# xyang9527/dro-sfm

Measured on AMD Instinct MI355X. Metric: training images/sec (KITTI 192x640 mf self-sup), higher is better.
Workload: dtype f32; 1 GPU; KITTI 192x640 mf self-sup (configs[1]); model=DepthPoseNet it8-seq4-inter-out, global_batch=2, per_gpu_batch=2, ref_frames=2, parallelism=dp1, optimizer=Adam lr 2e-4, execution=hipgraph, update_blocks=depth block + pose block (side stream, with both context encoders), encoder_3x3_s1=hip, encoder_strided=hip, exchange=none (world 1)

## Files before the change

dro-sfm_amd/csrc/conv.hip:

```cpp
#include <hip/hip_runtime.h>

#include <algorithm>
#include <climits>
#include <cstddef>
#include <cstdio>
#include <cstdlib>
#include <cstring>
#include <map>
#include <mutex>
#include <string>
#include <type_traits>

#include "conv_common.hpp"
#include "dro_common.hpp"
#include "wgrad_group_plan.hpp"

namespace dro {


template <int BM, int MODE, int ACT, int EPI>
__global__ __launch_bounds__(256) void igemm_kernel(IgArgs a) {
  constexpr int WM = BM / 32;
  constexpr int KSTEPS = (WM == 2) ? 16 : 8;
  __shared__ float Ws[2][kBK][BM + 1];
// ... 179 lines not shown
    if (old == n - 1u) __hip_atomic_store(c, 0u, __ATOMIC_RELAXED, __HIP_MEMORY_SCOPE_AGENT);
  }
  __syncthreads();
  return *flag != 0u;
}

__device__ __forceinline__ void bn_put(double2* p, double a, double b) {
  double* q = reinterpret_cast<double*>(p);
  __hip_atomic_store(q, a, __ATOMIC_RELAXED, __HIP_MEMORY_SCOPE_AGENT);
  __hip_atomic_store(q + 1, b, __ATOMIC_RELAXED, __HIP_MEMORY_SCOPE_AGENT);
}

__device__ __forceinline__ double2 bn_get(const double2* p) {
  double* q = const_cast<double*>(reinterpret_cast<const double*>(p));
  return make_double2(__hip_atomic_load(q, __ATOMIC_RELAXED, __HIP_MEMORY_SCOPE_AGENT),
                      __hip_atomic_load(q + 1, __ATOMIC_RELAXED, __HIP_MEMORY_SCOPE_AGENT));
}

__device__ __forceinline__ double2 bn_fold(const double2* base, int n, int rows, int r, int j, int T) {
  double s1 = 0.0, s2 = 0.0;
  for (int p0 = j; p0 < n; p0 += 8 * T) {
    double2 v[8];
#pragma unroll
    for (int u = 0; u < 8; ++u) {
      const int p = p0 + u * T;
      v[u] = p < n ? bn_get(base + (size_t)p * rows + r) : make_double2(0.0, 0.0);
    }
#pragma unroll
    for (int u = 0; u < 8; ++u) {
      s1 += v[u].x;
      s2 += v[u].y;
    }
  }
  for (int o = 1; o < T; o <<= 1) {
    s1 += __shfl_xor(s1, o);
    s2 += __shfl_xor(s2, o);
  }
  return make_double2(s1, s2);
}

template <int EPI>
__device__ __forceinline__ void bn_finalize_row(const BnFuse& f, int r, int rows, long long L, double s1, double s2) {
  if (EPI == 5) {
    const double mean = s1 / (double)L;
    double var = s2 / (double)L - mean * mean;
    var = var > 0.0 ? var : 0.0;
    const float invstd = (float)(1.0 / sqrt(var + (double)f.eps));
    const float mu = (float)mean;
    f.coef[r] = (f.gamma ? f.gamma[r] : 1.f) * invstd;
    f.coef[rows + r] = mu;
    f.coef[2 * rows + r] = f.beta ? f.beta[r] : 0.f;
    f.save_mean[r] = mu;
    f.save_invstd[r] = invstd;
    if (f.rmean) {
      const double unb = L > 1 ? var * (double)L / (double)(L - 1) : var;
      f.rmean[r] = (1.f - f.momentum) * f.rmean[r] + f.momentum * mu;
      f.rvar[r] = (1.f - f.momentum) * f.rvar[r] + f.momentum * (float)unb;
    }
    if (r == 0 && f.nbt) *f.nbt += 1;
  } else {
    const float invstd = f.invstd[r];
    f.coef[r] = (f.gamma ? f.gamma[r] : 1.f) * invstd;
    f.coef[rows + r] = (float)(s1 / (double)L);
    f.coef[2 * rows + r] = (float)(s2 / (double)L);
    f.coef[3 * rows + r] = f.mean[r];
    f.coef[4 * rows + r] = invstd;
    if (f.dgamma) f.dgamma[r] = (float)s2;
    if (f.dbeta) f.dbeta[r] = (float)s1;
  }
}

template <int EPI>
__device__ void bn_finish(const IgArgs& a, int pt, int rt, int row0, int bm) {
  __shared__ unsigned flag;
  const BnFuse& f = a.bn;
  if (f.dbg & 1) return;
  const int rows = a.rows, ptiles = a.g.B * a.tiles_img;
  const int grp = pt / f.g1, lo = grp * f.g1, n1 = min(f.g1, ptiles - lo);
  if (!last_arrival(f.cnt + (size_t)rt * f.ngroups + grp, (unsigned)n1, &flag)) return;
  const int T = (int)blockDim.x / bm, rl = (int)threadIdx.x / T, j = (int)threadIdx.x - rl * T;
  const int r = row0 + rl;
  const bool live = r < rows;
  {
    const double2 v = bn_fold(f.part + (size_t)lo * rows, live ? n1 : 0, rows, live ? r : 0, j, T);
    if (live && j == 0) bn_put(f.part2 + (size_t)grp * rows + r, v.x, v.y);
  }
  if (!last_arrival(f.cnt + (size_t)a.row_tiles * f.ngroups + rt, (unsigned)f.ngroups, &flag)) return;
  const double2 v = bn_fold(f.part2, live ? f.ngroups : 0, rows, live ? r : 0, j, T);
  if (!live || j != 0) return;
  bn_finalize_row<EPI>(f, r, rows, (long long)a.g.B * a.g.H * a.g.W, v.x, v.y);
}

template <int EPI>
__global__ __launch_bounds__(256) void bn_finalize_kernel(BnFuse f, int rows, int ptiles, long long L) {
  __shared__ double red[2][4];
  const int r = blockIdx.x;
  double s1 = 0.0, s2 = 0.0;
  for (int p = threadIdx.x; p < ptiles; p += 256) {
    const double2 v = f.part[(size_t)p * rows + r];
    s1 += v.x;
    s2 += v.y;
  }
#pragma unroll
  for (int o = 32; o > 0; o >>= 1) {
    s1 += __shfl_xor(s1, o);
    s2 += __shfl_xor(s2, o);
  }
  const int w = threadIdx.x >> 6;
  if ((threadIdx.x & 63) == 0) {
    red[0][w] = s1;
    red[1][w] = s2;
  }
  __syncthreads();
  if (threadIdx.x == 0)
    bn_finalize_row<EPI>(f, r, rows, L, (red[0][0] + red[0][1]) + (red[0][2] + red[0][3]),
                         (red[1][0] + red[1][1]) + (red[1][2] + red[1][3]));
}

template <int BM, int KH, int KW, int MODE, int ACT, int EPI, int KS, int XF = 0>
__global__ __launch_bounds__(256 * KS) void dconv_kernel(IgArgs a) {
  using S = HaloShape<BM, KH, KW>;
  {
    const unsigned long long t0 = __builtin_amdgcn_s_memtime();
    if (a.stamps && (threadIdx.x == 0 || threadIdx.x == blockDim.x - 64))
      a.stamps[(size_t)blockIdx.x * 16 + (threadIdx.x == 0 ? 10 : 11)] = t0;
  }
  constexpr int PF = KS <= 2 ? 2 : 1;
  static_assert(KS == 1 || S::LDS >= 4 * 16 * 64, "cross-group reduction area");
  constexpr int T = S::T, TH = S::TH, TW = S::TW, HWd = S::HWd, HALO = S::HALO, HPAD = S::HPAD;
  constexpr int CK = S::CK, NJ = S::NJ, XPER = CK / 4;
  constexpr int RUN = MODE == 0 ? S::RUN0 : S::RUN1, WS = MODE == 0 ? S::WS0 : S::WS1;
  constexpr int WSZ = MODE == 0 ? S::WSZ0 : S::WSZ1, STAGE = S::STAGE;
  constexpr int WM = BM / 32;
  constexpr int PH = KH / 2, PW = KW / 2;
  __shared__ float smem_all[KS * S::LDS];
  const int cb1 = a.cbase[1], cb2 = a.cbase[2], cb3 = a.cbase[3];
  const int H = a.g.H, W = a.g.W;
  const int Cin = a.g.Cin, Cout = a.g.Cout, rows = a.rows, kch = a.kch;
  const int CinT = Cin * T;
  const float* __restrict__ Wt = a.weight;
  const float* __restrict__ Gp = a.G;
  const int tid = threadIdx.x & 255, lane = tid & 63;
  const int grp = KS == 1 ? 0 : __builtin_amdgcn_readfirstlane(threadIdx.x >> 8);
  const int wave = __builtin_amdgcn_readfirstlane(tid >> 6);
  float* smem = smem_all + grp * S::LDS;
  const int tile = xcd_remap(blockIdx.x, gridDim.x);
  const int pt = (int)udiv((unsigned)tile, a.rt_div), rt = tile - pt * a.row_tiles;
  const int row0 = rt * BM;
  const int b = (int)udiv((unsigned)pt, a.ti_div), trem = pt - b * a.tiles_img;
  const int tyi = (int)udiv((unsigned)trem, a.tx_div);
  const int ty0 = tyi * TH, tx0 = (trem - tyi * a.tiles_x) * TW;
  const size_t HW = (size_t)H * W;
  const unsigned HWu = (unsigned)HW;
  const int nck = (kch + CK - 1) / CK;
  const int cbeg = blockIdx.y * a.chunks_per_split;
  const int cend = min(nck, cbeg + a.chunks_per_split);

  unsigned xpb[NJ];
  bool xok[NJ], own[NJ];
  static_assert(XF == 0 || ((MODE == 0) == (XF != 3) && ACT == 0), "BN staging transforms: XF 1/2 forward, 3 data gradient");
#pragma unroll
  for (int j = 0; j < NJ; ++j) {
    const int e = lane + 64 * j;
    const int hy = e / HWd, hx = e - hy * HWd;
    const int yy = ty0 - PH + hy, xx = tx0 - PW + hx;
    xok[j] = e < HALO && (unsigned)yy < (unsigned)H && (unsigned)xx < (unsigned)W;
    xpb[j] = xok[j] ? 4u * (unsigned)(yy * W + xx) : 0u;
    own[j] = XF != 0 && xok[j] && hy >= PH && hy < PH + TH && hx >= PW && hx < PW + TW;
  }
  const unsigned wlast = (unsigned)Cout * CinT - 1;

  unsigned long long sQ[4];
  unsigned sR[4], sM[4];
#pragma unroll
  for (int t = 0; t < 4; ++t) {
    if (MODE == 0) {
      sQ[t] = a.sq0[t] + (unsigned long long)b * a.sqb[t];
      sR[t] = a.sr[t];
      sM[t] = a.sm[t];
    } else {
      sQ[t] = reinterpret_cast<unsigned long long>(Gp) + 4ull * (unsigned long long)b * Cout * HW;
      sR[t] = 4u * HWu;
      sM[t] = ~0u;
    }
  }
  const unsigned long long dQ1 = sQ[1] - sQ[0], dQ2 = sQ[2] - sQ[1], dQ3 = sQ[3] - sQ[2];
  const unsigned dR1 = sR[1] - sR[0], dR2 = sR[2] - sR[1], dR3 = sR[3] - sR[2];
  const unsigned dM1 = sM[1] - sM[0], dM2 = sM[2] - sM[1], dM3 = sM[3] - sM[2];
  const long long sbase = MODE == 0 ? reinterpret_cast<long long>(a.src[0].p) : reinterpret_cast<long long>(Gp);
  const long long yshift = reinterpret_cast<long long>(XF == 2 ? a.bn.skip : XF == 3 ? a.bn.z : a.gy) - sbase;
  const long long oshift = reinterpret_cast<long long>(a.bn.yout) - sbase;

  constexpr bool FOLD = MODE == 1 && ACT != 0;
  constexpr bool Y2 = FOLD || XF == 2 || XF == 3;
  constexpr int NXC = XF == 3 ? 5 : 3;
  const float galpha = a.galpha;
  constexpr int W4 = S::WTOT / 4, WPER4 = (W4 + 255) / 256;
  constexpr int WREG = 4 * WPER4;
  static_assert(S::WTOT % 4 == 0 && RUN % 4 == 0, "float4 weight runs");
  unsigned woff[WPER4];
  int wdst[WPER4];
#pragma unroll
  for (int i = 0; i < WPER4; ++i) {
    const int e = 4 * (tid + 256 * i);
    const int run = e / RUN, rem = e - run * RUN;
    woff[i] = (unsigned)run * CinT + (unsigned)rem;
    wdst[i] = (W4 % 256 == 0 || e < S::WTOT) ? run * WS + rem : -1;
  }
  typedef __attribute__((address_space(1))) char* GWPtr;
  struct Stage {
    float xr[XPER * NJ], yr[Y2 ? XPER * NJ : 1], wv[WREG];
    unsigned cmask;
    unsigned ownc;
    float xc[XF ? NXC * XPER : 1];
    GWPtr yo[XF ? XPER : 1];
  };
  typedef __attribute__((address_space(1))) const char* GPtr;
  typedef __attribute__((address_space(1))) const float* GFPtr;
  struct Rows {
    unsigned gbase;
    GPtr rowp[XPER], yrow[XPER];
    unsigned M[XPER];
  };
  constexpr int NVM = WPER4 + XPER * NJ;
  auto prep = [&](Stage& st, int chunk, Rows& r) {
    const int c0 = chunk * CK;
    r.gbase = MODE == 0 ? (unsigned)row0 * CinT + (unsigned)c0 * T : (unsigned)c0 * CinT + (unsigned)row0 * T;
    unsigned cm = 0;
#pragma unroll
    for (int i = 0; i < XPER; ++i) {
      const int ch = c0 + wave * XPER + i;
      const bool cok = ch < kch;
      cm |= cok ? (1u << i) : 0u;
      const int cc = cok ? ch : 0;
      const unsigned long long k1 = MODE == 0 ? 0ull - (unsigned long long)(cc >= cb1) : 0ull;
      const unsigned long long k2 = MODE == 0 ? 0ull - (unsigned long long)(cc >= cb2) : 0ull;
      const unsigned long long k3 = MODE == 0 ? 0ull - (unsigned long long)(cc >= cb3) : 0ull;
      const unsigned j1 = (unsigned)k1, j2 = (unsigned)k2, j3 = (unsigned)k3;
      const unsigned long long Q = sQ[0] + (dQ1 & k1) + (dQ2 & k2) + (dQ3 & k3);
      const unsigned R = sR[0] + (dR1 & j1) + (dR2 & j2) + (dR3 & j3);
      r.M[i] = sM[0] + (dM1 & j1) + (dM2 & j2) + (dM3 & j3);
      const unsigned long long rq = Q + (unsigned long long)(unsigned)cc * R;
      r.rowp[i] = reinterpret_cast<GPtr>(rq);
      r.yrow[i] = reinterpret_cast<GPtr>(rq + (unsigned long long)yshift);
      if (XF) {
        st.yo[i] = reinterpret_cast<GWPtr>(rq + (unsigned long long)oshift);
#pragma unroll
        for (int k = 0; k < NXC; ++k) st.xc[k * XPER + i] = a.bn.xcoef[k * kch + cc];
      }
    }
    st.cmask = cm;
    if (XF) st.ownc = (unsigned)(chunk % a.row_tiles) == (unsigned)rt ? ~0u : 0u;
  };
  auto item = [&](Stage& st, const Rows& r, int k) {
    if (k < WPER4) {
      const unsigned g = r.gbase + woff[k];
      const float4 v = *reinterpret_cast<const float4*>(Wt + (g < wlast - 3 ? g : wlast - 3));
      st.wv[4 * k] = v.x;
      st.wv[4 * k + 1] = v.y;
      st.wv[4 * k + 2] = v.z;
      st.wv[4 * k + 3] = v.w;
    } else {
      const int q = k - WPER4, i = q / NJ, j = q - i * NJ;
      const unsigned o = xpb[j] & r.M[i];
      st.xr[q] = *reinterpret_cast<GFPtr>(r.rowp[i] + o);
      if (Y2) st.yr[q] = *reinterpret_cast<GFPtr>(r.yrow[i] + o);
    }
  };
  auto load = [&](Stage& st, int chunk) {
    Rows r;
    prep(st, chunk, r);
#pragma unroll
    for (int k = 0; k < NVM; ++k) item(st, r, k);
  };
  auto store = [&](const Stage& st, int buf) {
    const float(&xr)[XPER * NJ] = st.xr;
    const float(&yr)[Y2 ? XPER * NJ : 1] = st.yr;
    const float(&wv)[WREG] = st.wv;
    float* Ws = smem + buf * STAGE;
    float* Xs = Ws + WSZ + wave * XPER * HPAD + lane;
    auto xval = [&](int i, int j) {
      const bool ok = ((st.cmask >> i) & 1u) && xok[j];
      float v = ok ? xr[i * NJ + j] : 0.f;
      if (XF == 1 || XF == 2) {
        const float r = fmaf(v - st.xc[XPER + i], st.xc[i], st.xc[2 * XPER + i]) + (XF == 2 ? yr[i * NJ + j] : 0.f);
        v = ok ? fmaxf(r, 0.f) : 0.f;
      } else if (XF == 3) {
        const float xh = (yr[i * NJ + j] - st.xc[3 * XPER + i]) * st.xc[4 * XPER + i];
        const float r = st.xc[i] * (v - st.xc[XPER + i] - xh * st.xc[2 * XPER + i]);
        v = ok ? r : 0.f;
      }
      if (XF && own[j] && ((st.cmask & st.ownc) >> i & 1u)) *reinterpret_cast<__attribute__((address_space(1))) float*>(st.yo[i] + xpb[j]) = v;
      if (MODE == 1) v *= galpha;
      if (FOLD) v *= act_bwd(yr[i * NJ + j], ACT);
      return v;
    };
    constexpr int JF = NJ * 64 <= HPAD ? NJ : NJ - 1;
#pragma unroll
    for (int i = 0; i < XPER; ++i) {
#pragma unroll
      for (int j = 0; j < JF; ++j) Xs[i * HPAD + 64 * j] = xval(i, j);
    }
    if (JF < NJ && lane + 64 * (NJ - 1) < HPAD) {
#pragma unroll
      for (int i = 0; i < XPER; ++i) Xs[i * HPAD + 64 * (NJ - 1)] = xval(i, NJ - 1);
    }
#pragma unroll
    for (int i = 0; i < WPER4; ++i) {
      if (W4 % 256 == 0 || wdst[i] >= 0) {
        float* d = Ws + wdst[i];
        d[0] = wv[4 * i];
        d[1] = wv[4 * i + 1];
        d[2] = wv[4 * i + 2];
        d[3] = wv[4 * i + 3];
      }
    }
  };

  const int wr = (WM == 2) ? (wave & 1) : 0;
  const int wc = (WM == 2) ? (wave >> 1) : (wave & 1);
  const int wk = (WM == 2) ? 0 : (wave >> 1);
  const int q = wc * 32 + (lane & 31);
  const int qy = q / TW, qx = q - qy * TW;
  const int qoff = qy * HWd + qx;
  const int hi = lane >> 5;
  const int arow = wr * 32 + (lane & 31);
  constexpr int NS = (WM == 2) ? CK / 2 : CK / 4;
  const int s_lo = (WM == 2) ? 0 : wk * NS;
  constexpr int ASTEP = MODE == 0 ? 2 * T : 2 * WS;
  const int abase = (MODE == 0 ? arow * WS + hi * T : hi * WS + arow * T) + s_lo * ASTEP;
  const int bbase = hi * HPAD + qoff + 2 * s_lo * HPAD;
  f32x16 acc;
#pragma unroll
  for (int r = 0; r < 16; ++r) acc[r] = 0.f;

  const int nit = (cend - cbeg + KS - 1) / KS;
  auto chunk_of = [&](int it) { return cbeg + it * KS + grp; };
  unsigned long long* const stp = a.stamps ? a.stamps + (size_t)blockIdx.x * 16 : nullptr;
  auto stamp = [&](int k) {
    if (stp && threadIdx.x == 0 && k < 15) stp[k] = __builtin_amdgcn_s_memtime();
  };
  stamp(0);
  if (stp && threadIdx.x == blockDim.x - 64) stp[15] = __builtin_amdgcn_s_memtime();
  auto mma_ld = [&](int buf, Stage* st, const Rows* r) {
    const float* wa = smem + buf * STAGE + abase;
    const float* xb = smem + buf * STAGE + WSZ + bbase;
    constexpr int NMF = T * NS, PD = 2;
    auto aoff = [](int k) { return (k / NS) + (k % NS) * ASTEP; };
    auto boff = [](int k) {
      const int tap = k / NS, s = k % NS, ty = tap / KW, tx = tap % KW;
      return (MODE == 0 ? ty * HWd + tx : (KH - 1 - ty) * HWd + (KW - 1 - tx)) + 2 * s * HPAD;
    };
    float av[PD + 1], bv[PD + 1];
#pragma unroll
    for (int k = 0; k < PD && k < NMF; ++k) {
      av[k] = wa[aoff(k)];
      bv[k] = xb[boff(k)];
    }
#pragma unroll
    for (int k = 0; k < NMF; ++k) {
      if (k + PD < NMF) {
        av[(k + PD) % (PD + 1)] = wa[aoff(k + PD)];
        bv[(k + PD) % (PD + 1)] = xb[boff(k + PD)];
      }
      acc = mfma32(av[k % (PD + 1)], bv[k % (PD + 1)], acc);
      if (st) {
        if (k < NVM) item(*st, *r, k);
        __builtin_amdgcn_sched_barrier(0x0006);
      }
    }
    if (st) {
#pragma unroll
      for (int k = NMF; k < NVM; ++k) item(*st, *r, k);
    }
  };
  auto mma = [&](int buf) { mma_ld(buf, nullptr, nullptr); };
  Stage sa, sb;
  if (chunk_of(0) < cend) {
    load(sa, chunk_of(0));
    store(sa, 0);
  }
  stamp(12);
  if (PF == 2 && chunk_of(1) < cend) load(sb, chunk_of(1));
  __syncthreads();
  stamp(1);
  const int dbg = ablation_flags(a.dbg);
  if (PF == 1) {
    for (int it = 0; it < nit; ++it) {
      const int buf = it & 1;
      const bool more = chunk_of(it + 1) < cend;
      if (more && !(dbg & 3)) {
        Rows r;
        prep(sa, chunk_of(it + 1), r);
        mma_ld(buf, &sa, &r);
      } else {
        if (more && !(dbg & 1)) load(sa, chunk_of(it + 1));
        if ((KS == 1 || chunk_of(it) < cend) && !(dbg & 2)) mma(buf);
      }
      if (more && !(dbg & 4)) store(sa, buf ^ 1);
      __syncthreads();
      if (it < 8) stamp(2 + it);
    }
  } else {
    for (int it = 0; it < nit; it += 2) {
      if (chunk_of(it + 2) < cend) load(sa, chunk_of(it + 2));
      if (chunk_of(it) < cend) mma(0);
      if (chunk_of(it + 1) < cend) store(sb, 1);
      __syncthreads();
      if (it < 8) stamp(2 + it);
      if (it + 1 >= nit) break;
      if (chunk_of(it + 3) < cend) load(sb, chunk_of(it + 3));
      if (chunk_of(it + 1) < cend) mma(1);
      if (chunk_of(it + 2) < cend) store(sa, 0);
      __syncthreads();
      if (it < 7) stamp(3 + it);
    }
  }
  constexpr int NSET = (WM == 1 ? 2 : 1) * KS;
  static_assert(NSET * BM * 64 <= KS * S::LDS, "reduction sets fit in the staging LDS");
  {
    const int set = grp * (WM == 1 ? 2 : 1) + (WM == 1 ? wk : 0);
    float* red = smem_all + (size_t)set * BM * 64;
#pragma unroll
    for (int r = 0; r < 16; ++r) {
      const int rl = wr * 32 + (r & 3) + 8 * (r >> 2) + 4 * (lane >> 5);
      red[rl * 64 + wc * 32 + (lane & 31)] = acc[r];
    }
  }
  __syncthreads();
  stamp(13);
  const long long P = (long long)a.g.B * HW;
  if constexpr (EPI >= 5) {
    constexpr int NIT = BM * 64 / (256 * KS);
    float second[EPI == 6 ? NIT : 1];
#pragma unroll
    for (int it = 0; it < NIT; ++it) {
      const int e = (int)threadIdx.x + it * 256 * KS;
      const int rl = e >> 6, pl = e & 63;
      float v = 0.f;
#pragma unroll
      for (int g = 0; g < KS; ++g) {
        if (WM == 1)
          v += smem_all[((size_t)(2 * g) * BM + rl) * 64 + pl] + smem_all[((size_t)(2 * g + 1) * BM + rl) * 64 + pl];
        else
          v += smem_all[((size_t)g * BM + rl) * 64 + pl];
      }
      const int row = row0 + rl;
      const int py = pl / TW, px = pl - py * TW;
      const int oy = ty0 + py, ox = tx0 + px;
      float first = 0.f;
      if (EPI == 6) second[it] = 0.f;
      if (row < rows && oy < H && ox < W) {
        const size_t epix = (size_t)oy * W + ox;
        if (EPI == 5) {
          first = v + (a.bias ? a.bias[row] : 0.f);
          a.out[((size_t)b * a.out_ctot + a.out_coff + row) * HW + epix] = first;
        } else {
          const size_t idx = ((size_t)b * rows + row) * HW + epix;
          first = a.bn.y[idx] > 0.f ? v : 0.f;
          const float xh = (a.bn.z[idx] - a.bn.mean[row]) * a.bn.invstd[row];
          a.gsrc[0][idx] = first;
          second[it] = first * xh;
        }
      }
      smem_all[e] = first;
    }
    __syncthreads();
    const int rl = threadIdx.x, row = row0 + rl;
    const bool rowt = rl < BM && row < rows && !(a.bn.dbg & 4);
    double s1 = 0.0, s2 = 0.0;
    if (rowt) {
#pragma unroll 16
      for (int p = 0; p < 64; ++p) {
        const double v = smem_all[rl * 64 + p];
        s1 += v;
        if (EPI == 5) s2 += v * v;
      }
    }
    if (EPI == 6) {
      __syncthreads();
#pragma unroll
      for (int it = 0; it < NIT; ++it) smem_all[(int)threadIdx.x + it * 256 * KS] = second[EPI == 6 ? it : 0];
      __syncthreads();
      if (rowt) {
#pragma unroll 16
        for (int p = 0; p < 64; ++p) s2 += (double)smem_all[rl * 64 + p];
      }
    }
    if (rowt && !(a.bn.dbg & 2)) bn_put(a.bn.part + (size_t)pt * rows + row, s1, s2);
    if (a.bn.inkernel) bn_finish<EPI>(a, pt, rt, row0, BM);
    stamp(14);
    return;
  }
  for (int e = threadIdx.x; e < BM * 64; e += 256 * KS) {
    const int rl = e >> 6, pl = e & 63;
    float v = 0.f;
#pragma unroll
    for (int g = 0; g < KS; ++g) {
      if (WM == 1)
        v += smem_all[((size_t)(2 * g) * BM + rl) * 64 + pl] + smem_all[((size_t)(2 * g + 1) * BM + rl) * 64 + pl];
      else
        v += smem_all[((size_t)g * BM + rl) * 64 + pl];
    }
    const int row = row0 + rl;
    const int py = pl / TW, px = pl - py * TW;
    const int oy = ty0 + py, ox = tx0 + px;
    if (row >= rows || oy >= H || ox >= W) continue;
    const size_t epix = (size_t)oy * W + ox;
    if (a.part)
      a.part[(size_t)blockIdx.y * rows * P + (size_t)row * P + (size_t)b * HW + epix] = v;
    else
      epi_store<MODE, ACT, EPI>(a, row, b, epix, HW, v);
  }
  stamp(14);
}


__global__ __launch_bounds__(256) void wgrad_kernel(IgArgs a) {
  constexpr int NB = 1;
  __shared__ float Gs[NB][kWP][64 + 1];
  __shared__ float Xs[NB][kWP][64 + 1];
  const int cb1 = a.cbase[1], cb2 = a.cbase[2], cb3 = a.cbase[3];
  const int H = a.g.H, W = a.g.W, KW = a.g.KW, PH = a.g.PH, PW = a.g.PW;
  const int Hsrc = a.Hs, Wsrc = a.Ws, sh = a.sshift;
  const unsigned HWs = (unsigned)Hsrc * (unsigned)Wsrc;
  const int Cin = a.g.Cin, Cout = a.g.Cout;
  const float* __restrict__ Gp = a.G;
  const FastDiv cindiv = a.cindiv, kwdiv = a.kwdiv;
  const int tid = threadIdx.x, lane = tid & 63, wave = tid >> 6;
  const int t = blockIdx.x;
  const int ot = t % a.otiles, nt = t / a.otiles;
  const int o0 = ot * 64, n0 = nt * 64;
  const int NK = a.K;
  const int NC = a.gbias ? NK + 1 : NK;
  const size_t HW = (size_t)H * W;
  const unsigned HWu = (unsigned)HW;
  const long long P = (long long)a.g.B * HW;
  const long long pbeg = (long long)blockIdx.y * a.pchunk;
  const long long pend = pbeg + a.pchunk < P ? pbeg + a.pchunk : P;
  float gr[16], xr[16];
  unsigned gmask = 0, xmask = 0, omask = 0;

  auto load = [&](long long q0) {
    const long long p = q0 + lane;
    const bool v = p < pend;
    const int b = v ? (int)(p / (long long)HW) : 0;
    const int pix = v ? (int)(p - (long long)b * HW) : 0;
    const int py = pix / W, px = pix - py * W;
    gmask = 0;
    xmask = 0;
    omask = 0;
#pragma unroll
    for (int j = 0; j < 16; ++j) {
      const int o = o0 + wave * 16 + j;
      const bool gok = v && o < Cout;
      gmask |= gok ? (1u << j) : 0u;
      gr[j] = Gp[gok ? ((unsigned)b * Cout + o) * HWu + pix : 0u];
      const int n = __builtin_amdgcn_readfirstlane(n0 + wave * 16 + j);
      const bool nv = n < NK;
      const int tap = nv ? fdiv(n, cindiv) : 0, ch = nv ? n - tap * Cin : 0;
      const int ty = fdiv(tap, kwdiv), dy = ty - PH, dx = tap - ty * KW - PW;
      const int yy = (py << sh) + dy, xx = (px << sh) + dx;
      const bool ok = v && nv && (unsigned)yy < (unsigned)Hsrc && (unsigned)xx < (unsigned)Wsrc;
      const unsigned spix = (unsigned)(yy * Wsrc + xx);
      xmask |= ok ? (1u << j) : 0u;
      omask |= (v && n == NK) ? (1u << j) : 0u;
      const RowDesc d = row_desc(cb1, cb2, cb3, ch, HWs);
      const unsigned e = (unsigned)b * d.A + d.Bc + (d.M ? spix : 0u);
      xr[j] = d.p[ok ? e : 0u];
    }
  };
  auto store = [&](int buf) {
#pragma unroll
    for (int j = 0; j < 16; ++j) {
      Gs[buf][lane][wave * 16 + j] = (gmask >> j) & 1u ? gr[j] : 0.f;
      Xs[buf][lane][wave * 16 + j] = (xmask >> j) & 1u ? xr[j] : ((omask >> j) & 1u ? 1.f : 0.f);
    }
  };

  const int wo = wave & 1, wc = wave >> 1;
  f32x16 acc;
#pragma unroll
  for (int r = 0; r < 16; ++r) acc[r] = 0.f;
  if (pbeg < pend) {
    load(pbeg);
    store(0);
  }
  __syncthreads();
  int buf = 0;
  for (long long q0 = pbeg; q0 < pend; q0 += kWP) {
    const bool more = q0 + kWP < pend;
    if (more) load(q0 + kWP);
#pragma unroll
    for (int s = 0; s < kWP / 2; ++s) {
      const int kk = s * 2 + (lane >> 5);
      acc = mfma32(Gs[buf][kk][wo * 32 + (lane & 31)], Xs[buf][kk][wc * 32 + (lane & 31)], acc);
    }
    if (NB == 1) __syncthreads();
    if (more) store(NB == 1 ? 0 : buf ^ 1);
    __syncthreads();
    buf = NB == 1 ? 0 : buf ^ 1;
  }
  float* wp = a.part + (size_t)blockIdx.y * Cout * (NK + 1);
  const int n = n0 + wc * 32 + (lane & 31);
#pragma unroll
  for (int r = 0; r < 16; ++r) {
    const int o = o0 + wo * 32 + (r & 3) + 8 * (r >> 2) + 4 * (lane >> 5);
    if (o < Cout && n < NC) wp[(size_t)o * (NK + 1) + n] = acc[r];
  }
}

constexpr int kMaxUse = 16;
struct WgMulti {
  IgArgs a;
  int nuse;
  int use_tiles;
  Slice usrc[kMaxUse][kMaxSrc];
  const float* uG[kMaxUse];
  const float* uy[kMaxUse];
};

template <bool MULTI>
struct WgParam {
  typedef IgArgs T;
  static __device__ __forceinline__ const IgArgs& ig(const IgArgs& x) { return x; }
};
template <>
struct WgParam<true> {
  typedef WgMulti T;
  static __device__ __forceinline__ const IgArgs& ig(const WgMulti& x) { return x.a; }
};

typedef const float* FPtr;
typedef __attribute__((address_space(4))) const FPtr* KFPtr;

__device__ __forceinline__ __attribute__((address_space(4))) const char* kernarg_base() {
  return (__attribute__((address_space(4))) const char*)__builtin_amdgcn_kernarg_segment_ptr();
}

template <int KH, int KW>
struct HaloShapeW {
  static constexpr int T = KH * KW;
  static constexpr bool TAPSPLIT = T == 9;
  static constexpr int TPW = TAPSPLIT ? 5 : T;
  static constexpr int TH = HaloShape<32, KH, KW>::TH, TW = 64 / TH;
  static constexpr int HWd = TW + KW - 1;
  static constexpr int HALO = (TH + KH - 1) * HWd;
  static constexpr int HPAD = HALO | 1;
  static constexpr int NJ = (HALO + 63) / 64;
  static constexpr int BC = 32;
  static constexpr int GPAD = 65;
  static constexpr int STAGE = 64 * GPAD + BC * HPAD;
  static constexpr int LDS = 2 * STAGE > 2 * 16 * 64 * 2 ? 2 * STAGE : 2 * 16 * 64 * 2;
  static_assert(NJ <= 2 && TW % 2 == 0, "halo shape");
};

template <int KH, int KW, int GACT, bool MULTI>
__global__ __launch_bounds__(256) void wgrad_halo_kernel(typename WgParam<MULTI>::T P) {
  const IgArgs& a = WgParam<MULTI>::ig(P);
  using S = HaloShapeW<KH, KW>;
  constexpr int T = S::T, TH = S::TH, TW = S::TW, HWd = S::HWd, HALO = S::HALO, HPAD = S::HPAD;
// ... 1344 lines not shown
          }
        }
    }
  }
#pragma unroll
  for (int i = 0; i < CINP; ++i) red[(cg * 64 + px) * CINP + i] = acc[i];
  __syncthreads();
  const long long P = (long long)a.g.B * HW;
  for (int e = threadIdx.x; e < 64 * CINP; e += 256) {
    const int p = e / CINP, ci = e % CINP;
    if (ci >= Cin) continue;
    const float v = (red[(0 * 64 + p) * CINP + ci] + red[(1 * 64 + p) * CINP + ci]) +
                    (red[(2 * 64 + p) * CINP + ci] + red[(3 * 64 + p) * CINP + ci]);
    const int oy = ty0 + (p / 8), ox = tx0 + (p % 8);
    if (oy >= H || ox >= W) continue;
    const size_t epix = (size_t)oy * W + ox;
    if (a.part)
      a.part[(size_t)blockIdx.y * Cin * P + (size_t)ci * P + (size_t)b * HW + epix] = v;
    else
      grad_put(a.gsrc[0], a.gsrc_ctot[0], a.gsrc_coff[0], a.gsrc_acc[0], ci, b, epix, HW, v);
  }
}

bool g_conv_log = false;
std::mutex g_conv_log_mu;
std::map<std::string, std::pair<long long, double>> g_conv_log_map;

void conv_log(const char* name, double flops) {
  if (!g_conv_log) return;
  std::lock_guard<std::mutex> lk(g_conv_log_mu);
  auto& e = g_conv_log_map[name];
  e.first += 1;
  e.second += flops;
}

template <typename... Ts>
void conv_logf(double flops, const char* fmt, Ts... args) {
  if (!g_conv_log) return;
  char buf[160];
  snprintf(buf, sizeof(buf), fmt, args...);
  conv_log(buf, flops);
}

bool k7_ok(int KH, int KW, int Cin, int pad, int stride) {
  static const bool off = getenv("DRO_K7_WGRAD_OFF") != nullptr;
  return !off && KH == 7 && KW == 7 && pad == 3 &&
         ((stride == 2 && (Cin == 3 || Cin == 6)) || (stride == 1 && (Cin == 1 || Cin == 6)));
}

int k7_splits(int B, int Ho, int Wo) {
  static const int per = (int)env_int("DRO_K7_TILES_PER_BLOCK", 4);
  static const int cap = (int)env_int("DRO_K7_MAX_BLOCKS", 256);
  const int tiles = B * ((Ho + 7) / 8) * ((Wo + 7) / 8);
  int sp = (tiles + per - 1) / per;
  if (sp > cap) sp = cap;
  return sp < 1 ? 1 : sp;
}

size_t k7_part_bytes(int B, int Ho, int Wo, int Cin, int Cout) {
  return align256((size_t)k7_splits(B, Ho, Wo) * Cout * (Cin * 49 + 1) * sizeof(float));
}

int launch_wgrad_k7(IgArgs& a, int stride, int splits, hipStream_t s) {
  const int Cin = a.g.Cin, NK = Cin * 49;
  const int tiles = a.g.B * ((a.g.H + 7) / 8) * ((a.g.W + 7) / 8);
  if (splits > tiles) splits = tiles;
  if (splits < 1) splits = 1;
  const dim3 grid((unsigned)splits, (unsigned)((a.g.Cout + 63) / 64));
  conv_logf(2.0 * a.g.Cout * NK * (double)a.g.B * a.g.H * a.g.W, "wgrad_k7_kernel<%d, %d>", stride, Cin);
  static const int forced = env_int("DRO_K7_GROUPS", 0);
  const int groups = forced == 1 || forced == 2 ? forced : (stride == 2 && Cin == 3 ? 2 : 1);
#define DRO_K7(S_, C_, NW_, J_)                                                                         \
  do {                                                                                                  \
    if (groups == 2) hipLaunchKernelGGL((wgrad_k7_kernel<S_, C_, NW_, J_, 2>), grid, dim3(128 * NW_), 0, s, a); \
    else hipLaunchKernelGGL((wgrad_k7_kernel<S_, C_, NW_, J_, 1>), grid, dim3(64 * NW_), 0, s, a);     \
  } while (0)
  if (stride == 2 && Cin == 3) DRO_K7(2, 3, 5, 1);
  else if (stride == 2 && Cin == 6) DRO_K7(2, 6, 5, 2);
  else if (stride == 1 && Cin == 1) DRO_K7(1, 1, 2, 1);
  else if (stride == 1 && Cin == 6) DRO_K7(1, 6, 5, 2);
#undef DRO_K7
  else {
    set_error("wgrad_k7: unsupported channel count");
    return DRO_E_SHAPE;
  }
  int st = launch_status("wgrad_k7_kernel launch failed");
  if (st) return st;
  a.K = NK;
  launch_wgrad_finish(a, splits, s);
  return launch_status("wgrad_finish_kernel launch failed");
}

bool k7_fwd_ok(int KH, int KW, int Cin, int pad, int stride, int act, const float* bias) {
  static const bool on = env_int("DRO_K7_FWD", 0) != 0;
  return on && KH == 7 && KW == 7 && pad == 3 && stride == 2 && (Cin == 3 || Cin == 6) && act == 0 && !bias;
}

int launch_fwd_k7(IgArgs& a, hipStream_t s) {
  const int tiles = a.g.B * ((a.g.H + 7) / 8) * ((a.g.W + 7) / 8);
  static const int per = (int)env_int("DRO_K7_FWD_TILES_PER_BLOCK", 4);
  int nb = (tiles + per - 1) / per;
  if (nb < 1) nb = 1;
  const dim3 grid((unsigned)nb, (unsigned)((a.g.Cout + 63) / 64));
  conv_logf(2.0 * a.g.Cout * a.g.Cin * 49 * (double)a.g.B * a.g.H * a.g.W, "fwd_k7s2_kernel<%d>", a.g.Cin);
  if (a.g.Cin == 3) hipLaunchKernelGGL((fwd_k7s2_kernel<3>), grid, dim3(256), 0, s, a);
  else hipLaunchKernelGGL((fwd_k7s2_kernel<6>), grid, dim3(256), 0, s, a);
  return launch_status("fwd_k7s2_kernel launch failed");
}


template <int MODE, int EPI>
bool thin_ok(const IgArgs& a) {
  if (EPI != 0 || a.g.KH != kThinK || a.g.KW != kThinK || a.g.B > 65535) return false;
  const int cin = MODE == 0 ? a.g.Cin : a.rows;
  if (cin > 8 || a.cbase[1] < cin) return false;
  if (MODE == 1 && a.gsrc[0] == nullptr) return false;
  return true;
}

template <int MODE, int ACT>
int launch_thin(IgArgs& a, int max_splits, hipStream_t s) {
  const int tiles_x = (a.g.W + 7) / 8, tiles = tiles_x * ((a.g.H + 7) / 8);
  const double flops = 2.0 * a.rows * a.kch * a.g.KH * a.g.KW * (double)a.g.B * a.g.H * a.g.W;
  if (MODE == 0) {
    conv_logf(flops, "thin_fwd_kernel<%d>", ACT);
    hipLaunchKernelGGL((thin_fwd_kernel<ACT>), dim3(tiles, (a.g.Cout + 15) / 16, a.g.B), dim3(256), 0,
                       s, a, tiles_x);
    return launch_status("thin_fwd_kernel launch failed");
  }
  const int splits = max_splits >= 4 ? 4 : (max_splits >= 2 ? 2 : 1);
  const int cps = (a.g.Cout + splits - 1) / splits;
  if (splits == 1) a.part = nullptr;
  const dim3 grid(tiles, splits, a.g.B);
  conv_logf(flops, "thin_dgrad_kernel<%d, %d>", ACT, a.rows == 1 ? 1 : a.rows == 2 ? 2 : a.rows <= 4 ? 4 : 8);
  if (a.rows == 1)
    hipLaunchKernelGGL((thin_dgrad_kernel<ACT, 1>), grid, dim3(256), 0, s, a, tiles_x, cps);
  else if (a.rows == 2)
    hipLaunchKernelGGL((thin_dgrad_kernel<ACT, 2>), grid, dim3(256), 0, s, a, tiles_x, cps);
  else if (a.rows <= 4)
    hipLaunchKernelGGL((thin_dgrad_kernel<ACT, 4>), grid, dim3(256), 0, s, a, tiles_x, cps);
  else
    hipLaunchKernelGGL((thin_dgrad_kernel<ACT, 8>), grid, dim3(256), 0, s, a, tiles_x, cps);
  int st = launch_status("thin_dgrad_kernel launch failed");
  if (st || splits == 1) return st;
  const long long P = (long long)a.g.B * a.g.H * a.g.W;
  const long long total = (long long)a.rows * P;
  hipLaunchKernelGGL((igemm_finish_kernel<1, 0, 0>), dim3((unsigned)((total + 255) / 256)), dim3(256), 0,
                     s, a, splits);
  return launch_status("igemm_finish_kernel launch failed");
}

unsigned long long* g_conv_stamps = nullptr;

template <int MODE, int ACT, int EPI, int XF = 0>
int launch_igemm(IgArgs& a, long long P, char* ws, hipStream_t s) {
  IgPlan pl = a.flat_only ? plan_igemm_flat(a.rows, a.kch, a.g.KH, a.g.KW, a.g.B, a.g.H, a.g.W)
                          : plan_igemm(a.rows, a.kch, a.g.KH, a.g.KW, a.g.B, a.g.H, a.g.W);
  constexpr bool BNF = EPI >= 5 || XF != 0;
  if (BNF) {
    if (!pl.halo || a.g.KH != 3 || a.g.KW != 3 || a.flat_only) {
      set_error("conv2d: BatchNorm fusion needs a 3x3 stride-1 halo convolution");
      return DRO_E_SHAPE;
    }
    if (EPI >= 5) {
      pl.chunks_per_split = (a.kch + pl.CK - 1) / pl.CK;
      pl.ksplit = 1;
    }
  }
  a.stamps = g_conv_stamps;
  a.dbg = 0;
  if (g_conv_stamps) {
    const char* e = getenv("DRO_CONV_DBG");
    a.dbg = e ? atoi(e) : 0;
  }
  a.K = a.kch * a.g.KH * a.g.KW;
  static const bool thin_off = getenv("DRO_CONV_NO_THIN") != nullptr;
  if (!BNF && !a.flat_only && !thin_off && thin_ok<MODE, EPI>(a)) {
    a.part = reinterpret_cast<float*>(ws);
    return launch_thin<MODE, ACT>(a, pl.ksplit, s);
  }
  if constexpr (EPI < 3 && !BNF) {
    if (!a.flat_only && a.wsplit && xconv_supported(a.g.KH, a.g.KW)) return launch_xconv<MODE, ACT, EPI>(a, ws, s);
  }
  a.row_tiles = pl.row_tiles;
  a.chunks_per_split = pl.chunks_per_split;
  a.part = pl.ksplit > 1 ? reinterpret_cast<float*>(ws) : nullptr;
  const dim3 grid(pl.row_tiles * pl.ptiles, pl.ksplit);
  const double flops = 2.0 * a.rows * a.kch * a.g.KH * a.g.KW * (double)P;
  if (pl.halo)
    conv_logf(flops, "dconv_kernel<%d, %d, %d, %d, %d, %d, %d>", pl.bm, a.g.KH, a.g.KW, MODE, ACT, EPI, pl.kin);
  else
    conv_logf(flops, "igemm_kernel<%d, %d, %d, %d>", pl.bm, MODE, ACT, EPI);
  if (pl.halo) {
    a.TH = pl.TH;
    a.TW = pl.TW;
    a.HWd = pl.HWd;
    a.HPAD = pl.HPAD;
    a.tiles_x = pl.tiles_x;
    a.tiles_img = pl.tiles_img;
    a.CK = pl.CK;
    a.rt_div = make_div32(pl.row_tiles);
    a.ti_div = make_div32(pl.tiles_img);
    a.tx_div = make_div32(pl.tiles_x);
    if (MODE == 0) {
      const unsigned long long HWl = (unsigned long long)a.g.H * a.g.W;
      for (int t = 0; t < kMaxSrc; ++t) {
        const Slice& sl = a.src[t];
        const unsigned long long chs = sl.bcast ? 1ull : HWl;
        const long long cbt = t == 0 ? 0 : a.cbase[t];
        a.sq0[t] = reinterpret_cast<unsigned long long>(sl.p) +
                   4ull * (unsigned long long)(((long long)sl.coff - cbt) * (long long)chs);
        a.sqb[t] = 4ull * (unsigned long long)sl.ctot * chs;
        a.sr[t] = 4u * (unsigned)chs;
        a.sm[t] = sl.bcast ? 0u : ~0u;
      }
    }
    const int KH = a.g.KH;
    const int KW = a.g.KW;
#define DRO_DCONV(BM_, KH_, KW_)                                                                    \
    do {                                                                                            \
      if (pl.kin == 4)                                                                              \
        hipLaunchKernelGGL((dconv_kernel<BM_, KH_, KW_, MODE, ACT, EPI, 4, XF>), grid, dim3(1024), 0, s, a); \
      else if (pl.kin == 2)                                                                         \
        hipLaunchKernelGGL((dconv_kernel<BM_, KH_, KW_, MODE, ACT, EPI, 2, XF>), grid, dim3(512), 0, s, a);  \
      else                                                                                          \
        hipLaunchKernelGGL((dconv_kernel<BM_, KH_, KW_, MODE, ACT, EPI, 1, XF>), grid, dim3(256), 0, s, a);  \
    } while (0)
    if constexpr (BNF) {
      if (pl.bm == 32) DRO_DCONV(32, 3, 3);
      else DRO_DCONV(64, 3, 3);
    } else if (pl.bm == 32) {
      if (KH == 1 && KW == 1) DRO_DCONV(32, 1, 1);
      else if (KH == 1) DRO_DCONV(32, 1, 5);
      else if (KW == 1) DRO_DCONV(32, 5, 1);
      else DRO_DCONV(32, 3, 3);
    } else {
      if (KH == 1 && KW == 1) DRO_DCONV(64, 1, 1);
      else if (KH == 1) DRO_DCONV(64, 1, 5);
      else if (KW == 1) DRO_DCONV(64, 5, 1);
      else DRO_DCONV(64, 3, 3);
    }
#undef DRO_DCONV
  } else if constexpr (!BNF) {
    a.kdiv = make_fdiv(a.kch);
    if (pl.bm == 64)
      hipLaunchKernelGGL((igemm_kernel<64, MODE, ACT, EPI>), grid, dim3(256), 0, s, a);
    else
      hipLaunchKernelGGL((igemm_kernel<32, MODE, ACT, EPI>), grid, dim3(256), 0, s, a);
  }
  int st = launch_status("conv kernel launch failed");
  if (st || (EPI < 5 && pl.ksplit == 1)) return st;
  if constexpr (EPI >= 5) {
    if (st || a.bn.inkernel) return st;
    hipLaunchKernelGGL((bn_finalize_kernel<EPI>), dim3((unsigned)a.rows), dim3(256), 0, s, a.bn, a.rows,
                       pl.ptiles, P);
    return launch_status("bn_finalize_kernel launch failed");
  } else {
    const long long total = (long long)a.rows * P;
    long long blocks = (total + 255) / 256;
    if (blocks > 2048) blocks = 2048;
    hipLaunchKernelGGL((igemm_finish_kernel<MODE, ACT, EPI>), dim3((unsigned)blocks), dim3(256), 0, s, a,
                       pl.ksplit);
    return launch_status("igemm_finish_kernel launch failed");
  }
}

int check_ws(const void* ws, size_t have, size_t need, const char* what) {
  if (need > 0 && (!ws || have < need)) {
    static thread_local char msg[192];
    snprintf(msg, sizeof(msg), "%s: workspace of %zu bytes is smaller than the %zu required "
             "(dro_conv2d_workspace_bytes)", what, ws ? have : (size_t)0, need);
    set_error(msg);
    return DRO_E_SHAPE;
  }
  return DRO_OK;
}

}

#define DRO_ACT_SWITCH(act, ...)                  \
  switch (act) {                                  \
    case 0: { constexpr int A_ = 0; __VA_ARGS__; } break; \
    case 1: { constexpr int A_ = 1; __VA_ARGS__; } break; \
    case 2: { constexpr int A_ = 2; __VA_ARGS__; } break; \
    case 3: { constexpr int A_ = 3; __VA_ARGS__; } break; \
    default: set_error("conv2d: unknown activation"); return DRO_E_MODE; \
  }

extern "C" int dro_conv2d_plan(int rows, int kch, int KH, int KW, int B, int H, int W, long long* info) {
  if (!info || rows < 1 || kch < 1 || KH < 1 || KW < 1 || B < 1 || H < 1 || W < 1) {
    set_error("conv2d_plan: bad arguments");
    return DRO_E_SHAPE;
  }
  const IgPlan pl = plan_igemm(rows, kch, KH, KW, B, H, W);
  const long long v[16] = {pl.halo, pl.bm, pl.row_tiles, pl.ptiles, pl.ksplit, pl.chunks_per_split,
                           pl.TH, pl.TW, pl.HWd, pl.HPAD, pl.tiles_x, pl.tiles_img, pl.CK,
                           (long long)pl.lds_bytes, (long long)pl.part_bytes, pl.kin};
  for (int i = 0; i < 16; ++i) info[i] = v[i];
  return DRO_OK;
}

extern "C" int dro_conv_log(int enable) {
  std::lock_guard<std::mutex> lk(g_conv_log_mu);
  g_conv_log = enable != 0;
  if (enable) g_conv_log_map.clear();
  return DRO_OK;
}

extern "C" long long dro_conv_log_read(char* buf, long long cap) {
  std::lock_guard<std::mutex> lk(g_conv_log_mu);
  std::string out;
  for (const auto& kv : g_conv_log_map) {
    char line[256];
    snprintf(line, sizeof(line), "%s\t%lld\t%.17g\n", kv.first.c_str(), kv.second.first, kv.second.second);
    out += line;
  }
  const long long n = (long long)out.size();
  if (buf && cap > 0) {
    const long long m = n < cap - 1 ? n : cap - 1;
    memcpy(buf, out.data(), (size_t)m);
    buf[m] = 0;
  }
  return n;
}

extern "C" int dro_debug_conv_stamps(void* buffer) {
  g_conv_stamps = static_cast<unsigned long long*>(buffer);
  return DRO_OK;
}

extern "C" size_t dro_conv2d_workspace_bytes(int B, int H, int W, int Cin, int Cout, int KH, int KW) {
  if (B < 1 || H < 1 || W < 1 || Cin < 1 || Cout < 1 || KH < 1 || KW < 1) return 0;
  const size_t f = fwd_workspace(B, H, W, Cin, Cout, KH, KW);
  const size_t b = bwd_workspace(B, H, W, Cin, Cout, KH, KW);
  return f > b ? f : b;
}

extern "C" int dro_conv2d_forward(const dro_slice* srcs, int nsrc, const float* weight, const float* bias,
                                  int B, int H, int W, int Cout, int KH, int KW, int act, float alpha,
                                  float* out, int out_ctot, int out_coff, const void* wsplit,
                                  void* workspace, size_t workspace_bytes, void* stream) {
// ... 151 lines not shown
  return launch_status("bn_bwd_coef_apply_kernel launch failed");
}

extern "C" int dro_bn_apply(const float* x, const float* skip, int relu, int B, int C, int H, int W,
                            const void* state, float* y, void* stream) {
  if (!bn_dims_ok(B, H, W, C, C) || (long long)B * C > 65535) {
    set_error("bn_apply: sizes out of range");
    return DRO_E_SHAPE;
  }
  if (!x || !y || !state) {
    set_error("bn_apply: NULL x/y/state");
    return DRO_E_NULL;
  }
  if (relu != 0 && relu != 1) {
    set_error("bn_apply: relu must be 0 or 1");
    return DRO_E_MODE;
  }
  const int HW = H * W;
  const float* coef = bn_coef(state, bn_layout(B, H, W, C));
  long long per = (2048 + (long long)B * C - 1) / ((long long)B * C);
  const long long need = (HW + 1023) / 1024;
  if (per > need) per = need;
  if (per < 1) per = 1;
  const dim3 grid((unsigned)per, (unsigned)(B * C));
  auto al = [](const void* p) { return p == nullptr || (reinterpret_cast<size_t>(p) & 15) == 0; };
  hipStream_t s = (hipStream_t)stream;
  if ((HW & 3) == 0 && al(x) && al(skip) && al(y))
    hipLaunchKernelGGL(bn_coef_apply_kernel<true>, grid, dim3(256), 0, s, x, skip, coef, relu, C, HW, y);
  else
    hipLaunchKernelGGL(bn_coef_apply_kernel<false>, grid, dim3(256), 0, s, x, skip, coef, relu, C, HW, y);
  return launch_status("bn_coef_apply_kernel launch failed");
}

extern "C" int dro_conv2d_bn_forward(const float* x, int B, int H, int W, int Cin, const float* weight, int Cout,
                                     const void* in_state, const float* in_skip, float* in_y,
                                     const dro_bn_params* bn, void* out_state, float* out, void* workspace,
                                     size_t workspace_bytes, void* stream) {
  if (!bn_dims_ok(B, H, W, Cin, Cout)) {
    set_error("conv2d_bn_forward: sizes out of range");
    return DRO_E_SHAPE;
  }
  if (!x || !weight || !out || (!in_state) != (!in_y) || (in_skip && !in_state) || (!bn) != (!out_state) ||
      (bn && (!bn->save_mean || !bn->save_invstd || (!bn->running_mean) != (!bn->running_var)))) {
    set_error("conv2d_bn_forward: NULL pointer (x/weight/out; in_y with in_state; out_state and "
              "save_mean/save_invstd with bn)");
    return DRO_E_NULL;
  }
  const dro_slice sl{x, Cin, Cin, 0, 0};
  IgArgs a = {};
  int st = conv_setup_geom(a, &sl, 1, B, H, W, Cout, 3, 3);
  if (st) return st;
  if ((st = check_ws(workspace, workspace_bytes, fwd_workspace(B, H, W, Cin, Cout, 3, 3), "conv2d_bn_forward")))
    return st;
  a.weight = weight;
  a.alpha = 1.f;
  a.out = out;
  a.out_ctot = Cout;
  a.out_coff = 0;
  a.rows = Cout;
  a.kch = Cin;
  if (in_state) {
    a.bn.xcoef = bn_coef(in_state, bn_layout(B, H, W, Cin));
    a.bn.skip = in_skip;
    a.bn.yout = in_y;
  }
  if (bn) {
    bn_bind(a.bn, out_state, bn_layout(B, H, W, Cout));
    a.bn.gamma = bn->gamma;
    a.bn.beta = bn->beta;
    a.bn.rmean = bn->running_mean;
    a.bn.rvar = bn->running_var;
    a.bn.nbt = bn->num_batches_tracked;
    a.bn.eps = bn->eps;
    a.bn.momentum = bn->momentum;
    a.bn.save_mean = bn->save_mean;
    a.bn.save_invstd = bn->save_invstd;
  }
  const long long P = (long long)B * H * W;
  hipStream_t s = (hipStream_t)stream;
  char* ws = static_cast<char*>(workspace);
  const int xf = in_state ? (in_skip ? 2 : 1) : 0;
  if (bn) {
    if (xf == 2) return launch_igemm<0, 0, 5, 2>(a, P, ws, s);
    if (xf == 1) return launch_igemm<0, 0, 5, 1>(a, P, ws, s);
    return launch_igemm<0, 0, 5, 0>(a, P, ws, s);
  }
  if (xf == 2) return launch_igemm<0, 0, 0, 2>(a, P, ws, s);
  if (xf == 1) return launch_igemm<0, 0, 0, 1>(a, P, ws, s);
  return launch_igemm<0, 0, 0, 0>(a, P, ws, s);
}

extern "C" int dro_conv2d_bn_backward_data(const float* weight, int B, int H, int W, int Cin, int Cout,
                                           const float* dout, const void* gin_state, const float* gin_z,
                                           float* gin_dz, const dro_bn_grad_params* src_bn, void* src_state,
                                           float* grad_x, int grad_x_accumulate, void* workspace,
                                           size_t workspace_bytes, void* stream) {
  if (!bn_dims_ok(B, H, W, Cin, Cout)) {
    set_error("conv2d_bn_backward_data: sizes out of range");
    return DRO_E_SHAPE;
  }
  if (!weight || !dout || !grad_x || (gin_state && (!gin_z || !gin_dz)) || (!src_bn) != (!src_state) ||
      (src_bn && (!src_bn->y || !src_bn->z || !src_bn->save_mean || !src_bn->save_invstd))) {
    set_error("conv2d_bn_backward_data: NULL pointer (weight/dout/grad_x; gin_z/gin_dz with gin_state; "
              "src_state and y/z/save_mean/save_invstd with src_bn)");
    return DRO_E_NULL;
  }
  if (src_bn && grad_x_accumulate) {
    set_error("conv2d_bn_backward_data: grad_x receives g with src_bn (no accumulation)");
    return DRO_E_MODE;
  }
  if (gin_state && src_bn) {
    set_error("conv2d_bn_backward_data: gin_state and src_bn in one call are not supported");
    return DRO_E_MODE;
  }
  const dro_slice sl{grad_x, Cin, Cin, 0, 0};
  IgArgs a = {};
  int st = conv_setup_geom(a, &sl, 1, B, H, W, Cout, 3, 3);
  if (st) return st;
  if ((st = check_ws(workspace, workspace_bytes, plan_igemm(Cin, Cout, 3, 3, B, H, W).part_bytes,
                     "conv2d_bn_backward_data")))
    return st;
  a.weight = weight;
  a.G = dout;
  a.galpha = 1.f;
  a.gsrc[0] = grad_x;
  a.gsrc_ctot[0] = Cin;
  a.gsrc_coff[0] = 0;
  a.gsrc_acc[0] = grad_x_accumulate ? 1 : 0;
  a.rows = Cin;
  a.kch = Cout;
  if (gin_state) {
    a.bn.xcoef = bn_coef(gin_state, bn_layout(B, H, W, Cout));
    a.bn.z = gin_z;
    a.bn.yout = gin_dz;
  }
  if (src_bn) {
    bn_bind(a.bn, src_state, bn_layout(B, H, W, Cin));
    a.bn.y = src_bn->y;
    a.bn.z = src_bn->z;
    a.bn.gamma = src_bn->gamma;
    a.bn.mean = src_bn->save_mean;
    a.bn.invstd = src_bn->save_invstd;
    a.bn.dgamma = src_bn->grad_gamma;
    a.bn.dbeta = src_bn->grad_beta;
  }
  const long long P = (long long)B * H * W;
  hipStream_t s = (hipStream_t)stream;
  char* ws = static_cast<char*>(workspace);
  if (src_bn) return launch_igemm<1, 0, 6, 0>(a, P, ws, s);
  if (gin_state) return launch_igemm<1, 0, 0, 3>(a, P, ws, s);
  return launch_igemm<1, 0, 0, 0>(a, P, ws, s);
}

extern "C" int dro_convgru_gates_forward(const dro_slice* srcs, int nsrc, const float* weight,
                                         const float* bias, int B, int H, int W, int hd, int KH, int KW,
                                         float* zr, float* rh, const void* wsplit, void* workspace,
                                         size_t workspace_bytes, void* stream) {
  IgArgs a = {};
  a.wsplit = static_cast<const char*>(wsplit);
  int st = conv_setup_geom(a, srcs, nsrc, B, H, W, 2 * hd, KH, KW);
  if (st) return st;
  if (!weight || !zr || !rh) {
    set_error("convgru_gates_forward: NULL weight/zr/rh");
    return DRO_E_NULL;
  }
  if (srcs[0].channels != hd || srcs[0].broadcast) {
    set_error("convgru_gates_forward: source 0 must be the dense hidden state (hd channels)");
    return DRO_E_SHAPE;
  }
  if ((st = check_ws(workspace, workspace_bytes, fwd_workspace(B, H, W, a.g.Cin, 2 * hd, KH, KW),
                     "convgru_gates_forward")))
    return st;
  a.weight = weight;
  a.bias = bias;
  a.alpha = 1.f;
  a.out = zr;
  a.out_ctot = 2 * hd;
  a.out_coff = 0;
  a.h = to_slice(srcs);
  a.aux = rh;
  a.hd = hd;
  a.rows = 2 * hd;
  a.kch = a.g.Cin;
  return launch_igemm<0, 2, 2>(a, (long long)B * H * W, static_cast<char*>(workspace), (hipStream_t)stream);
}

extern "C" int dro_convgru_blend_forward(const dro_slice* srcs, int nsrc, const float* weight,
                                         const float* bias, int B, int H, int W, int Cout, int KH, int KW,
                                         const dro_slice* z, const dro_slice* h, float* q_out, float* out,
                                         int out_ctot, int out_coff, const void* wsplit, void* workspace,
                                         size_t workspace_bytes, void* stream) {
  IgArgs a = {};
  a.wsplit = static_cast<const char*>(wsplit);
  int st = conv_setup_geom(a, srcs, nsrc, B, H, W, Cout, KH, KW);
  if (st) return st;
  if (!weight || !out || !q_out || !z || !h || !z->data || !h->data) {
    set_error("convgru_blend_forward: NULL weight/out/q/z/h");
    return DRO_E_NULL;
  }
  if ((st = check_ws(workspace, workspace_bytes, fwd_workspace(B, H, W, a.g.Cin, Cout, KH, KW),
                     "convgru_blend_forward")))
    return st;
  a.weight = weight;
  a.bias = bias;
  a.alpha = 1.f;
  a.out = out;
  a.out_ctot = out_ctot;
  a.out_coff = out_coff;
  a.z = to_slice(z);
  a.h = to_slice(h);
  a.aux = q_out;
  a.rows = Cout;
  a.kch = a.g.Cin;
  return launch_igemm<0, 3, 1>(a, (long long)B * H * W, static_cast<char*>(workspace),
                               (hipStream_t)stream);
}

struct GruFold {
  int kind;
  const float* zr;
  const float* h;
  float* dzr;
  float* dh;
  const float* q;
  float* dq;
  int dh_acc;
};

static int conv2d_backward_impl(const dro_slice* srcs, int nsrc, const float* weight, int B, int H, int W,
                                int Cout, int KH, int KW, int act, float alpha, const dro_slice* y,
                                const float* dout, float* const* grad_srcs, const int* grad_ctot,
                                const int* grad_coff, const int* grad_accumulate, float* grad_weight,
                                float* grad_bias, int grad_weight_accumulate, const void* wsplit,
                                void* workspace, size_t workspace_bytes, void* stream, const GruFold* gf) {
  IgArgs a = {};
  a.wsplit = static_cast<const char*>(wsplit);
  int st = conv_setup_geom(a, srcs, nsrc, B, H, W, Cout, KH, KW);
  if (st) return st;
  const bool pre = act != 0 || alpha != 1.f;
  if (!weight || !dout || (act != 0 && (!y || !y->data))) {
    set_error("conv2d_backward: NULL weight/dout/y");
    return DRO_E_NULL;
  }
  if (act < 0 || act > 3) {
    set_error("conv2d_backward: unknown activation");
    return DRO_E_MODE;
  }
  if (grad_bias && !grad_weight) {
    set_error("conv2d_backward: grad_bias requires grad_weight");
    return DRO_E_NULL;
  }
  if ((st = check_ws(workspace, workspace_bytes, bwd_workspace(B, H, W, a.g.Cin, Cout, KH, KW),
                     "conv2d_backward")))
    return st;
  for (int i = 0; i < nsrc; ++i) {
    a.gsrc[i] = grad_srcs ? grad_srcs[i] : nullptr;
    a.gsrc_ctot[i] = grad_ctot ? grad_ctot[i] : srcs[i].channels;
    a.gsrc_coff[i] = grad_coff ? grad_coff[i] : 0;
    a.gsrc_acc[i] = grad_accumulate ? grad_accumulate[i] : 0;
    if (a.gsrc[i] && too_big(B, a.gsrc_ctot[i], (long long)H * W)) {
      set_error("conv2d_backward: gradient target too large (32-bit offsets)");
      return DRO_E_SHAPE;
    }
  }
  if (gf && gf->kind == 3) {
    if (!gf->zr || !gf->h || !gf->dzr || !gf->dh) {
      set_error("convgru_candidate_backward: NULL zr/h/dzr/dh");
      return DRO_E_NULL;
    }
    if (srcs[0].channels != Cout || act != 0 || alpha != 1.f || grad_weight || too_big(B, 2 * Cout, (long long)H * W)) {
      set_error("convgru_candidate_backward: source 0 must be r*h with Cout channels (no activation, no weight gradient)");
      return DRO_E_SHAPE;
    }
    a.z = Slice{gf->zr, Cout, 2 * Cout, Cout, 0};
    a.h = Slice{gf->h, Cout, Cout, 0, 0};
    a.aux = gf->dzr;
    a.hd = Cout;
    a.gsrc[0] = gf->dh;
    a.gsrc_ctot[0] = Cout;
    a.gsrc_coff[0] = 0;
    a.gsrc_acc[0] = 1;
    a.wsplit = nullptr;
  } else if (gf) {
    const int hd = Cout / 2;
    if (!gf->zr || !gf->h || !gf->dzr || !gf->dh || !gf->q || !gf->dq || !a.gsrc[0]) {
      set_error("convgru_gates_backward: NULL zr/h/q/dq/dzr/dh or d h target");
      return DRO_E_NULL;
    }
    if (Cout % 2 || srcs[0].channels != hd || act != 0 || alpha != 1.f || grad_weight ||
        a.gsrc_ctot[0] != hd || a.gsrc_coff[0] != 0 || too_big(B, Cout, (long long)H * W)) {
      set_error("convgru_gates_backward: source 0 must be h with Cout / 2 channels and a dense d h target "
                "(no activation, no weight gradient)");
      return DRO_E_SHAPE;
    }
    a.z = Slice{gf->zr, hd, Cout, 0, 0};
    a.h = Slice{gf->h, hd, hd, 0, 0};
    a.aux = gf->dzr;
    a.hd = hd;
    a.g1q = gf->q;
    a.g1dq = gf->dq;
    a.g1dh = gf->dh;
    a.g1acc = gf->dh_acc ? 1 : 0;
    a.gsrc_acc[0] = 1;
    a.wsplit = nullptr;
  }
  a.weight = weight;
  a.gweight = grad_weight;
  a.gbias = grad_bias;
  a.wacc = grad_weight_accumulate ? 1 : 0;
  hipStream_t s = (hipStream_t)stream;
  const size_t HW = (size_t)H * W;
  const long long P = (long long)B * HW;
  const int T = KH * KW;
  char* ws = static_cast<char*>(workspace);
  char* ws_pre = ws;
  char* ws_ig = ws_pre + align256((size_t)Cout * P * sizeof(float));
  char* ws_wg = ws_ig + std::max(plan_igemm(a.g.Cin, Cout, KH, KW, B, H, W).part_bytes,
                                 xconv_part_bytes(a.g.Cin, Cout, KH, KW, B, H, W));
  const WhPlan wh = plan_wgrad_halo(a.g.Cin, Cout, KH, KW, B, H, W);
  const bool halo_dgrad = plan_igemm(a.g.Cin, Cout, KH, KW, B, H, W).halo;
  static const bool thin_off = getenv("DRO_CONV_NO_THIN") != nullptr;
  const bool thin_dgrad = KH == kThinK && KW == kThinK && nsrc == 1 && a.g.Cin <= 8 && B <= 65535 && !thin_off;
  const bool fold = pre && (halo_dgrad || thin_dgrad) && (wh.ok || !grad_weight) &&
                    (act == 0 || (y->total_channels == Cout && y->channel_offset == 0));
  a.galpha = fold ? alpha : 1.f;
  a.gy = (fold && act) ? y->data : nullptr;
  if (pre && !fold) {
    if ((long long)B * Cout > 65535 || HW >= ((size_t)1 << 31)) {
      set_error("conv2d_backward: B * Cout or H * W out of range for the gradient pre-pass");
      return DRO_E_SHAPE;
    }
    float* G = reinterpret_cast<float*>(ws_pre);
    hipLaunchKernelGGL(grad_pre_kernel, dim3((unsigned)((HW + 255) / 256), (unsigned)(B * Cout)), dim3(256), 0, s,
                       act, alpha, Cout, (int)HW, dout, to_slice(y), G);
    if ((st = launch_status("grad_pre_kernel launch failed"))) return st;
    a.G = G;
  } else {
    a.G = dout;
  }
  bool any_dgrad = false;
  for (int i = 0; i < nsrc; ++i) any_dgrad |= a.gsrc[i] != nullptr;
  if (any_dgrad) {
    a.rows = a.g.Cin;
    a.kch = Cout;
    const int gact = fold ? act : 0;
    if (gf && gf->kind == 3)
      st = launch_igemm<1, 0, 3>(a, P, ws_ig, s);
    else if (gf)
      st = launch_igemm<1, 0, 4>(a, P, ws_ig, s);
    else
      DRO_ACT_SWITCH(gact, st = (launch_igemm<1, A_, 0>(a, P, ws_ig, s)));
    if (st) return st;
  }
  if (grad_weight && wh.ok && !wgrad_v1()) {
    const WhPlan w2 = plan_wgrad2(a.g.Cin, Cout, KH, KW, 0, B, H, W);
    a.otiles = w2.otiles;
    a.tiles_x = w2.tiles_x;
    a.tiles_img = w2.tiles_img;
    a.chunks_per_split = w2.tiles_per_split;
    a.part = reinterpret_cast<float*>(ws_wg);
    a.bpart = reinterpret_cast<float*>(ws_wg + align256((size_t)w2.splits * Cout * a.g.Cin * T * sizeof(float)));
    const dim3 grid((unsigned)(w2.otiles * w2.ctiles * w2.tgroups), (unsigned)w2.splits);
    const int gact = fold ? act : 0;
    conv_logf(2.0 * Cout * a.g.Cin * T * (double)P, "wgrad2_kernel<%d, %d, %d, false, %d>", KH, KW, gact,
              w2.tgroups);
#define DRO_WG2(KH_, KW_, TG_) DRO_ACT_SWITCH(gact, hipLaunchKernelGGL((wgrad2_kernel<KH_, KW_, A_, false, TG_>), grid, dim3(512), 0, s, a))
    if (KH == 1 && KW == 1) { DRO_WG2(1, 1, 1); }
    else if (KH == 1) { DRO_WG2(1, 5, 1); }
// ... 646 lines not shown
```

dro-sfm_amd/csrc/conv_common.hpp:

```cpp
#pragma once
#include <hip/hip_runtime.h>

#include <cstddef>

#include "dro_common.hpp"

namespace dro {

typedef float f32x16 __attribute__((ext_vector_type(16)));

constexpr int kBN = 64;
constexpr int kBK = 32;
constexpr int kWP = 64;
constexpr int kMaxSrc = 4;

struct Slice {
  const float* p;
  int C, ctot, coff;
  int bcast;
};

struct FastDiv {
  unsigned m;
  int one;
};
__device__ __forceinline__ int fdiv(int n, FastDiv f) {
  return f.one ? n : (int)__umulhi((unsigned)n, f.m);
}

struct Div32 {
  unsigned m, d;
};
__device__ __forceinline__ unsigned udiv(unsigned n, Div32 f) {
  unsigned q = __umulhi(n, f.m);
  unsigned r = n - q * f.d;
  if (r >= f.d) {
    ++q;
    r -= f.d;
  }
  if (r >= f.d) ++q;
  return q;
}

struct ConvGeom {
  int B, H, W, Cin, Cout, KH, KW, PH, PW;
};

struct BnFuse {
  double2* part;
  double2* part2;
  unsigned* cnt;
  int g1, ngroups;
  const float* gamma;
  const float* beta;
  float* rmean;
  float* rvar;
  long long* nbt;
  float eps, momentum;
  float* save_mean;
  float* save_invstd;
  float* coef;
  const float* y;
  const float* z;
  const float* mean;
  const float* invstd;
  float* dgamma;
  float* dbeta;
  const float* xcoef;
  const float* skip;
  float* yout;
  int inkernel;
  int dbg;
};

struct IgArgs {
  ConvGeom g;
  Slice src[kMaxSrc];
  int cbase[kMaxSrc];
  const float* weight;
  const float* bias;
  float alpha;
  float* out;
  int out_ctot, out_coff;
  Slice z, h;
  float* aux;
  int hd;
  const float* g1q;
  float* g1dq;
  float* g1dh;
  int g1acc;
  const float* G;
  const float* gy;
  float galpha;
  float* gsrc[kMaxSrc];
  int gsrc_ctot[kMaxSrc], gsrc_coff[kMaxSrc], gsrc_acc[kMaxSrc];
  float* gweight;
  float* gbias;
  int wacc;
  int rows;
  int kch;
  int K;
  FastDiv kdiv, kwdiv, cindiv;
  int row_tiles;
  int chunks_per_split;
  float* part;
  float* bpart;
  int otiles;
  long long pchunk;
  int TH, TW, HWd, HPAD, tiles_x, tiles_img, CK;
  Div32 rt_div, ti_div, tx_div;
  unsigned long long sq0[kMaxSrc], sqb[kMaxSrc];
  unsigned sr[kMaxSrc], sm[kMaxSrc];
  const char* wsplit;
  unsigned long long wplane;
  unsigned wrow;
  int Hs, Ws, sshift;
  int flat_only;
  int pclass;
  long long pcmax;
  unsigned long long* stamps;
  int dbg;
  BnFuse bn;
};

#ifndef DRO_CONV_ABLATE
#define DRO_CONV_ABLATE 0
#endif
__device__ __forceinline__ int ablation_flags(int dbg) { return DRO_CONV_ABLATE ? dbg : 0; }

__device__ __forceinline__ float act_fwd(float v, int act) {
  switch (act) {
    case 1: return fmaxf(v, 0.f);
    case 2: return 1.f / (1.f + expf(-v));
    case 3: return tanhf(v);
    default: return v;
  }
}

__device__ __forceinline__ float act_bwd(float y, int act) {
  switch (act) {
    case 1: return y > 0.f ? 1.f : 0.f;
    case 2: return y * (1.f - y);
    case 3: return 1.f - y * y;
    default: return 1.f;
  }
}

__device__ __forceinline__ f32x16 mfma32(float a, float b, f32x16 c) {
  return __builtin_amdgcn_mfma_f32_32x32x2f32(a, b, c, 0, 0, 0);
}

__device__ __forceinline__ int xcd_remap(int id, int total) {
  const int xcd = id & 7, local = id >> 3, per = total >> 3, rem = total & 7;
  return (xcd < rem ? xcd * (per + 1) : rem * (per + 1) + (xcd - rem) * per) + local;
}

typedef __attribute__((address_space(4))) const Slice* KSlice;

__device__ __forceinline__ KSlice kernarg_srcs() {
  return (KSlice)((__attribute__((address_space(4))) const char*)__builtin_amdgcn_kernarg_segment_ptr() +
                  offsetof(IgArgs, src));
}

struct RowDesc {
  const float* p;
  unsigned A, Bc;
  bool M;
};

__device__ __forceinline__ RowDesc row_desc_at(KSlice base, int cb1, int cb2, int cb3, int ch,
                                               unsigned HW) {
  const int si = (ch >= cb1) + (ch >= cb2) + (ch >= cb3);
  const KSlice ks = base + si;
  const int cl = ch - (si == 0 ? 0 : si == 1 ? cb1 : si == 2 ? cb2 : cb3);
  const int ctot = ks->ctot, coff = ks->coff, bc = ks->bcast;
  RowDesc d;
  d.p = ks->p;
  d.A = bc ? (unsigned)ctot : (unsigned)ctot * HW;
  d.Bc = bc ? (unsigned)(coff + cl) : (unsigned)(coff + cl) * HW;
  d.M = !bc;
  return d;
}

__device__ __forceinline__ RowDesc row_desc(int cb1, int cb2, int cb3, int ch, unsigned HW) {
  return row_desc_at(kernarg_srcs(), cb1, cb2, cb3, ch, HW);
}

__device__ __forceinline__ void grad_put(float* dst, int ctot, int coff, int accf, int cl, int eb,
                                         size_t epix, size_t HW, float v) {
  if (!dst) return;
  float* q = dst + ((size_t)eb * ctot + coff + cl) * HW + epix;
  *q = accf ? (*q + v) : v;
}

template <int MODE, int ACT, int EPI>
__device__ __forceinline__ void epi_store(const IgArgs& a, int row, int eb, size_t epix, size_t HW,
                                          float acc) {
  if (MODE == 0) {
    float v = acc + (a.bias ? a.bias[row] : 0.f);
    v = a.alpha * act_fwd(v, ACT);
    if (EPI == 1) {
      const float z = a.z.p[((size_t)eb * a.z.ctot + a.z.coff + row) * HW + epix];
      const float hv = a.h.p[((size_t)eb * a.h.ctot + a.h.coff + row) * HW + epix];
      a.aux[((size_t)eb * a.rows + row) * HW + epix] = v;
      v = (1.f - z) * hv + z * v;
    }
    if (EPI == 2 && row >= a.hd) {
      const int c = row - a.hd;
      const float hv = a.h.p[((size_t)eb * a.h.ctot + a.h.coff + c) * HW + epix];
      a.aux[((size_t)eb * a.hd + c) * HW + epix] = v * hv;
    }
    a.out[((size_t)eb * a.out_ctot + a.out_coff + row) * HW + epix] = v;
  } else {
    if (EPI == 4 && row < a.cbase[1]) {
      float* q = a.gsrc[0] + ((size_t)eb * a.gsrc_ctot[0] + a.gsrc_coff[0] + row) * HW + epix;
      const float gn = *q + acc;
      *q = gn;
      const size_t zi = ((size_t)eb * a.z.ctot + a.z.coff + row) * HW + epix;
      const size_t i1 = ((size_t)eb * a.hd + row) * HW + epix;
      const float z = a.z.p[zi], qv = a.g1q[i1], hv = a.h.p[((size_t)eb * a.h.ctot + a.h.coff + row) * HW + epix];
      a.g1dq[i1] = gn * z * (1.f - qv * qv);
      a.aux[zi] = gn * (qv - hv) * z * (1.f - z);
      a.g1dh[i1] = a.g1acc ? a.g1dh[i1] + gn * (1.f - z) : gn * (1.f - z);
    } else if (EPI == 3 && row < a.cbase[1]) {
      const size_t zi = ((size_t)eb * a.z.ctot + a.z.coff + row) * HW + epix;
      const size_t hi = ((size_t)eb * a.h.ctot + a.h.coff + row) * HW + epix;
      const float r = a.z.p[zi];
      a.aux[zi] = acc * a.h.p[hi] * r * (1.f - r);
      float* q = a.gsrc[0] + ((size_t)eb * a.gsrc_ctot[0] + a.gsrc_coff[0] + row) * HW + epix;
      *q += acc * r;
    } else if (row < a.cbase[1])
      grad_put(a.gsrc[0], a.gsrc_ctot[0], a.gsrc_coff[0], a.gsrc_acc[0], row, eb, epix, HW, acc);
    else if (row < a.cbase[2])
      grad_put(a.gsrc[1], a.gsrc_ctot[1], a.gsrc_coff[1], a.gsrc_acc[1], row - a.cbase[1], eb, epix, HW, acc);
    else if (row < a.cbase[3])
      grad_put(a.gsrc[2], a.gsrc_ctot[2], a.gsrc_coff[2], a.gsrc_acc[2], row - a.cbase[2], eb, epix, HW, acc);
    else
      grad_put(a.gsrc[3], a.gsrc_ctot[3], a.gsrc_coff[3], a.gsrc_acc[3], row - a.cbase[3], eb, epix, HW, acc);
  }
}

template <int MODE, int ACT, int EPI>
__device__ __forceinline__ void epi_tile(const IgArgs& a, const f32x16& acc, int rbase, int eb,
                                         size_t epix, size_t HW) {
  const int rows = a.rows;
  if (MODE == 0) {
    float bv[16], zv[EPI == 1 ? 16 : 1], hv[EPI != 0 ? 16 : 1];
#pragma unroll
    for (int r = 0; r < 16; ++r) {
      const int row = rbase + (r & 3) + 8 * (r >> 2);
      const int rr = row < rows ? row : 0;
      bv[r] = a.bias ? a.bias[rr] : 0.f;
      if (EPI == 1) {
        zv[r] = a.z.p[((size_t)eb * a.z.ctot + a.z.coff + rr) * HW + epix];
        hv[r] = a.h.p[((size_t)eb * a.h.ctot + a.h.coff + rr) * HW + epix];
      }
      if (EPI == 2) {
        const int c = rr >= a.hd ? rr - a.hd : 0;
        hv[r] = a.h.p[((size_t)eb * a.h.ctot + a.h.coff + c) * HW + epix];
      }
    }
#pragma unroll
    for (int r = 0; r < 16; ++r) {
      const int row = rbase + (r & 3) + 8 * (r >> 2);
      if (row >= rows) continue;
      float v = acc[r] + bv[r];
      v = a.alpha * act_fwd(v, ACT);
      if (EPI == 1) {
        a.aux[((size_t)eb * a.rows + row) * HW + epix] = v;
        v = (1.f - zv[r]) * hv[r] + zv[r] * v;
      }
      if (EPI == 2 && row >= a.hd)
        a.aux[((size_t)eb * a.hd + (row - a.hd)) * HW + epix] = v * hv[r];
      a.out[((size_t)eb * a.out_ctot + a.out_coff + row) * HW + epix] = v;
    }
// ... 113 lines not shown
```

dro-sfm_amd/hip/_lib.py:

```python
import ctypes
import os

import torch

_HERE = os.path.dirname(os.path.abspath(__file__))
LIB_PATH = os.environ.get("DRO_LIB_PATH") or os.path.normpath(os.path.join(_HERE, "..", "libdro_amd.so"))

_c_float_p = ctypes.c_void_p
_lib = None


def _sig(fn, *argtypes, restype=ctypes.c_int):
    fn.argtypes = list(argtypes)
    fn.restype = restype


def load():
    global _lib
    if _lib is not None:
        return _lib
    if not os.path.exists(LIB_PATH):
        raise RuntimeError(
            f"dro_sfm_amd: native library not found at {LIB_PATH}; build it with "
            "`make -C dro-sfm_amd/csrc` (or __graft_entry__.build()).  There is no CPU fallback.")
    lib = ctypes.CDLL(LIB_PATH, mode=ctypes.RTLD_GLOBAL)
    P, I, F, S, Z = ctypes.c_void_p, ctypes.c_int, ctypes.c_float, ctypes.c_void_p, ctypes.c_size_t
    LL = ctypes.c_longlong
    _sig(lib.dro_last_error, restype=ctypes.c_char_p)
    _sig(lib.dro_abi_version)
    _sig(lib.dro_timestamp, P, I, S)
    _sig(lib.dro_wall_clock_hz, P)
    _sig(lib.dro_warp_cost_forward, P, P, P, I, F, F, P, P, F, P, I, I, I, I, I, I, I, I, P, S)
    _sig(lib.dro_warp_cost_workspace_bytes, I, I, I, I, restype=Z)
    _sig(lib.dro_warp_cost_backward, P, P, P, I, F, F, P, P, F, P, I, I, I, I, I, I, I, I,
         P, P, P, P, P, I, P, P, S)
    _sig(lib.dro_view_synthesis_forward, P, P, I, F, F, P, P, F, P, I, I, I, I, I, I, P, S)
    _sig(lib.dro_view_synthesis_backward, P, P, I, F, F, P, P, F, P, I, I, I, I, I, I, P, P, P, P, P, P, S)
    _sig(lib.dro_plane_sweep_forward, P, P, P, I, F, F, P, P, F, P, I, I, I, I, I, P, S)
    _sig(lib.dro_photometric_workspace_bytes, I, I, I, I, I, F, restype=Z)
    _sig(lib.dro_photometric_forward, P, P, P, P, P, P, I, I, I, I, I, I, F, F, F, F, I, I, F,
         P, P, S)
    _sig(lib.dro_photometric_clip_offset, I, I, I, I, I, I, restype=Z)
    _sig(lib.dro_photometric_backward, P, P, P, P, P, P, I, I, I, I, I, I, F, F, F, F, I, I, F,
         P, P, P, P, P, P, S)
    _sig(lib.dro_supervised_workspace_bytes, I, I, I, I, I, restype=Z)
    _sig(lib.dro_supervised_forward, P, P, P, P, P, P, I, I, I, I, I, I, F, F, P, P, S)
    _sig(lib.dro_supervised_backward, P, P, P, P, P, P, I, I, I, I, I, I, F, F, P, P, P, P, S)
    _sig(lib.dro_convex_upsample_forward, P, P, I, I, I, I, F, F, P, S)
    _sig(lib.dro_convex_upsample_backward, P, P, P, I, I, I, I, F, P, P, S)
    _sig(lib.dro_convex_upsample_many_forward, P, P, I, I, I, I, I, F, F, P, S)
    _sig(lib.dro_convex_upsample_many_workspace_bytes, I, I, I, I, restype=Z)
    _sig(lib.dro_convex_upsample_many_backward, P, P, P, I, I, I, I, I, F, P, P, P, Z, S)
    _sig(lib.dro_bilinear_upsample2x_forward, P, ctypes.c_longlong, I, I, P, S)
    _sig(lib.dro_bilinear_upsample2x_backward, P, ctypes.c_longlong, I, I, P, S)
    _sig(lib.dro_maxpool3x3s2_forward, P, ctypes.c_longlong, I, I, P, P, S)
    _sig(lib.dro_maxpool3x3s2_backward, P, P, ctypes.c_longlong, I, I, P, S)
    _sig(lib.dro_depth_metrics_blocks, I, I)
    _sig(lib.dro_depth_metrics_workspace_bytes, I, restype=Z)
    _sig(lib.dro_depth_metrics_prepare, P, P, I, I, I, I, I, F, F, I, I, I, I, P, P, P, S)
    _sig(lib.dro_depth_metrics_reduce, P, P, P, I, I, I, F, F, I, I, I, I, P, P, S)
    _sig(lib.dro_depth_metrics_median_workspace_bytes, I, restype=Z)
    _sig(lib.dro_depth_metrics_median, P, P, I, I, I, P, P, S)
    _sig(lib.dro_pose_mean_forward, P, P, P, I, I, I, F, S)
    _sig(lib.dro_pose_mean_backward, P, P, I, I, I, F, S)
    _sig(lib.dro_conv2d_strided_workspace_bytes, I, I, I, I, I, I, I, I, I, restype=Z)
    _sig(lib.dro_conv2d_strided_forward, P, P, P, I, I, I, I, I, I, I, I, I, I, P, P, Z, S)
    _sig(lib.dro_conv2d_strided_backward, P, P, P, I, I, I, I, I, I, I, I, I, P, I, P, P, I, P, Z, S)
    _sig(lib.dro_depth_metrics_demon_prepare, P, P, P, LL, I, I, I, I, I, F, F, P, P, P, S)
    _sig(lib.dro_depth_metrics_demon_reduce, P, P, P, P, LL, I, I, I, F, F, P, P, S)
    _sig(lib.dro_post_process_inv_depth, P, P, I, I, I, I, P, P, P, S)
    _sig(lib.dro_resize_rgb8_to_tensor, P, I, I, I, I, I, P, P, I, P, P, I, P, P, S)
    _sig(lib.dro_color_jitter_rgb8, P, I, I, I, P, P, S)
    _sig(lib.dro_resize_rgb8, P, I, I, I, I, I, P, P, I, P, P, I, P, P, S)
    _sig(lib.dro_rgb8_to_tensor, P, I, I, I, P, S)
    _sig(lib.dro_png_filtered_bytes, I, I, I, restype=Z)
    _sig(lib.dro_png_decode, P, P, I, I, I, I, P, P, P, S)
    _sig(lib.dro_batchnorm_workspace_bytes, I, I, I, restype=Z)
    _sig(lib.dro_batchnorm_relu_forward, P, P, P, P, I, I, I, I, F, F, P, P, P, P, P, P, P, Z, S)
    _sig(lib.dro_batchnorm_relu_backward, P, P, P, P, P, P, I, I, I, I, P, P, P, P, P, Z, S)
    _sig(lib.dro_conv2d_workspace_bytes, I, I, I, I, I, I, I, restype=Z)
    _sig(lib.dro_conv2d_plan, I, I, I, I, I, I, I, P)
    _sig(lib.dro_debug_conv_stamps, P)
    _sig(lib.dro_conv_log, I)
    _sig(lib.dro_conv_log_read, ctypes.c_char_p, ctypes.c_longlong, restype=ctypes.c_longlong)
    _sig(lib.dro_weight_split_bytes, I, I, I, I, I, restype=Z)
    _sig(lib.dro_weight_split, P, I, I, I, I, P, P, S)
    _sig(lib.dro_conv2d_forward, P, I, P, P, I, I, I, I, I, I, I, F, P, I, I, P, P, Z, S)
    _sig(lib.dro_convgru_gates_forward, P, I, P, P, I, I, I, I, I, I, P, P, P, P, Z, S)
    _sig(lib.dro_convgru_blend_forward, P, I, P, P, I, I, I, I, I, I, P, P, P, P, I, I, P, P, Z, S)
    _sig(lib.dro_conv2d_backward, P, I, P, I, I, I, I, I, I, I, F, P, P, P, P, P, P, P, P, I, P, P, Z, S)
    _sig(lib.dro_conv2d_weight_grad_multi_workspace_bytes, I, I, I, I, I, I, I, I, restype=Z)
    _sig(lib.dro_conv2d_weight_grad_multi, P, I, I, I, I, I, I, I, I, I, F, P, P, I, P, Z, S)
    _sig(lib.dro_conv2d_weight_grad_group_capacity, P, P)
    _sig(lib.dro_conv2d_weight_grad_group_workspace_bytes, P, I, I, I, restype=Z)
    _sig(lib.dro_conv2d_weight_grad_group, P, I, I, I, I, P, Z, S)
    _sig(lib.dro_adam_step, P, P, P, P, ctypes.c_longlong, P, P, S)
    _sig(lib.dro_gru_backward_elem, I, I, I, I, I, P, P, P, P, P, P, P, P, S)
    _sig(lib.dro_convgru_candidate_backward, P, I, P, I, I, I, I, I, I, P, P, P, P, P, P, P, P, P, P, Z, S)
    _sig(lib.dro_convgru_gates_backward, P, I, P, I, I, I, I, I, I, P, P, P, P, P, P, P, P, P, P, P, I, P, Z, S)
    _sig(lib.dro_bn_state_bytes, I, I, I, I, restype=Z)
    _sig(lib.dro_bn_apply, P, P, I, I, I, I, I, P, P, S)
    _sig(lib.dro_bn_backward_apply, P, P, I, I, I, I, P, P, S)
    _sig(lib.dro_conv2d_bn_forward, P, I, I, I, I, P, I, P, P, P, P, P, P, P, Z, S)
    _sig(lib.dro_conv2d_bn_backward_data, P, I, I, I, I, I, P, P, P, P, P, P, P, I, P, Z, S)
    _lib = lib
    return lib


EXPORTED = (
    "dro_last_error", "dro_abi_version", "dro_timestamp", "dro_wall_clock_hz",
    "dro_warp_cost_forward", "dro_warp_cost_workspace_bytes", "dro_warp_cost_backward",
    "dro_view_synthesis_forward", "dro_view_synthesis_backward",
    "dro_plane_sweep_forward",
    "dro_photometric_workspace_bytes", "dro_photometric_clip_offset", "dro_photometric_forward", "dro_photometric_backward",
    "dro_supervised_workspace_bytes", "dro_supervised_forward", "dro_supervised_backward",
    "dro_convex_upsample_forward", "dro_convex_upsample_backward",
    "dro_convex_upsample_many_forward", "dro_convex_upsample_many_workspace_bytes",
    "dro_convex_upsample_many_backward",
    "dro_bilinear_upsample2x_forward", "dro_bilinear_upsample2x_backward",
    "dro_maxpool3x3s2_forward", "dro_maxpool3x3s2_backward",
    "dro_depth_metrics_blocks", "dro_depth_metrics_workspace_bytes", "dro_depth_metrics_prepare",
    "dro_depth_metrics_reduce", "dro_depth_metrics_median_workspace_bytes", "dro_depth_metrics_median",
    "dro_depth_metrics_demon_prepare", "dro_depth_metrics_demon_reduce", "dro_post_process_inv_depth",
    "dro_conv2d_strided_workspace_bytes", "dro_conv2d_strided_forward", "dro_conv2d_strided_backward",
    "dro_pose_mean_forward", "dro_pose_mean_backward",
    "dro_resize_rgb8_to_tensor", "dro_color_jitter_rgb8", "dro_resize_rgb8", "dro_rgb8_to_tensor",
    "dro_png_filtered_bytes", "dro_png_decode",
    "dro_batchnorm_workspace_bytes", "dro_batchnorm_relu_forward", "dro_batchnorm_relu_backward",
    "dro_weight_split_bytes", "dro_weight_split",
    "dro_conv2d_workspace_bytes", "dro_conv2d_plan", "dro_debug_conv_stamps", "dro_conv_log", "dro_conv_log_read", "dro_conv2d_forward", "dro_convgru_gates_forward",
    "dro_convgru_blend_forward", "dro_conv2d_backward",
    "dro_conv2d_weight_grad_multi_workspace_bytes", "dro_conv2d_weight_grad_multi",
    "dro_conv2d_weight_grad_group_capacity", "dro_conv2d_weight_grad_group_workspace_bytes",
    "dro_conv2d_weight_grad_group",
    "dro_gru_backward_elem", "dro_convgru_candidate_backward", "dro_convgru_gates_backward", "dro_adam_step",
    "dro_bn_state_bytes", "dro_bn_apply", "dro_bn_backward_apply", "dro_conv2d_bn_forward", "dro_conv2d_bn_backward_data",
)


def check(status, what):
    if status != 0:
        msg = load().dro_last_error().decode(errors="replace")
        raise RuntimeError(f"{what} failed (status {status}): {msg}")


def ptr(t):
    return ctypes.c_void_p(t.data_ptr()) if t is not None else ctypes.c_void_p(0)


def stream_of(t):
    return ctypes.c_void_p(torch.cuda.current_stream(t.device).cuda_stream)


def require_device(*tensors, what="op"):
    for t in tensors:
        if t is None:
            continue
        if not t.is_cuda:
            raise RuntimeError(f"dro_sfm_amd.{what}: tensors must live on a ROCm device "
                               "(no CPU fallback)")
        if t.dtype != torch.float32:
            raise RuntimeError(f"dro_sfm_amd.{what}: expected float32, got {t.dtype}")
```

dro-sfm_amd/hip/conv.py:

```python
import contextlib
import ctypes
import os
from typing import Optional

import torch

from . import _lib
from ._lib import check, ptr, require_device, stream_of
from .ops import _sink_of

ACT = {None: 0, "none": 0, "relu": 1, "sigmoid": 2, "tanh": 3}


class DroSlice(ctypes.Structure):
    _fields_ = [("data", ctypes.c_void_p), ("channels", ctypes.c_int),
                ("total_channels", ctypes.c_int), ("channel_offset", ctypes.c_int),
                ("broadcast", ctypes.c_int)]


def _slice(t):
    B, C, H, W = t.shape
    s0, s1, s2, s3 = t.stride()
    if s2 == 0 and s3 == 0 and s1 == 1:
        return DroSlice(t.data_ptr(), C, s0 if B > 1 else C, 0, 1)
# ... 534 lines not shown

@torch.library.custom_op("dro::conv2d_strided_backward", mutates_args=("grad_x", "grad_weight", "grad_bias"))
def _conv2d_strided_bwd_op(x: Tensor, weight: Tensor, grad_out: Tensor, stride: int, pad: int,
                           grad_x: Optional[Tensor], grad_weight: Optional[Tensor], grad_bias: Optional[Tensor],
                           weight_accumulate: int, grad_x_accumulate: int = 0) -> None:
    lib = _lib.load()
    B, Cin, Hi, Wi = x.shape
    Cout, _, KH, KW = weight.shape
    nws = int(lib.dro_conv2d_strided_workspace_bytes(B, Hi, Wi, Cin, Cout, KH, KW, stride, pad))
    ws = torch.empty(max(nws, 1), dtype=torch.uint8, device=x.device)
    check(lib.dro_conv2d_strided_backward(ptr(x.contiguous()), ptr(weight.contiguous()), ptr(grad_out.contiguous()),
                                          B, Hi, Wi, Cin, Cout, KH, KW, stride, pad, ptr(grad_x), int(grad_x_accumulate),
                                          ptr(grad_weight),
                                          ptr(grad_bias), weight_accumulate, ptr(ws), nws, stream_of(grad_out)),
          "dro_conv2d_strided_backward")


@_conv2d_strided_bwd_op.register_fake
def _(x, weight, grad_out, stride, pad, grad_x, grad_weight, grad_bias, weight_accumulate, grad_x_accumulate=0):
    return None


def _conv2d_strided_setup(ctx, inputs, output):
    x, weight, bias, stride, pad, act = inputs
    ctx.save_for_backward(x, weight)
    has_bias = bias is not None
    ctx.meta = (stride, pad, act, has_bias, x.requires_grad, weight.requires_grad,
                has_bias and bias.requires_grad)
    ctx.direct = _direct_targets((weight,), (bias,) if has_bias else (), mark=False, in_setup=True)
    ctx.xsink = _sink_of(x) if x.requires_grad else None


def _conv2d_strided_backward(ctx, gout):
    x, weight = ctx.saved_tensors
    stride, pad, act, has_bias, need_x, need_w, need_b = ctx.meta
    if act:
        raise RuntimeError("conv2d_strided: backward through a fused activation is not supported")
    Cout = weight.shape[0]
    xacc = 0
    if ctx.xsink is not None:
        gx, xacc = ctx.xsink.target()
    else:
        gx = torch.empty_like(x) if need_x else None
    direct = ctx.direct
    if direct is not None:
        gw, gb, wacc = direct[2], direct[3] if has_bias else None, 1
    else:
        gw = torch.empty_like(weight) if need_w else None
        gb = torch.empty(Cout, device=x.device) if (has_bias and need_b) else None
        wacc = 0
    if gw is None and gb is not None:
        gw = torch.empty_like(weight)
    torch.ops.dro.conv2d_strided_backward(x, weight, gout, stride, pad, gx, gw, gb, wacc, xacc)
    if ctx.xsink is not None:
        gx = None
    if direct is not None:
        return gx, None, None, None, None, None
    return gx, (gw if need_w else None), (gb if has_bias and need_b else None), None, None, None


torch.library.register_autograd("dro::conv2d_strided", _conv2d_strided_backward, setup_context=_conv2d_strided_setup)


def conv2d_strided(x, weight, bias=None, stride=2, padding=1, act=None):
    _direct_targets((weight,), (bias,) if bias is not None else ())
    return torch.ops.dro.conv2d_strided(x, weight, bias, int(stride), int(padding), ACT[act])


@torch.library.custom_op("dro::gru_backward_elem", mutates_args=("dq", "dzr", "dh"))
def _gru_elem_op(stage: int, dhn: Optional[Tensor], zr: Tensor, q: Optional[Tensor], h: Tensor,
                 drh: Optional[Tensor], dq: Optional[Tensor], dzr: Tensor, dh: Tensor) -> None:
    lib = _lib.load()
    B, hd, H, W = h.shape
    check(lib.dro_gru_backward_elem(stage, B, hd, H, W, ptr(dhn), ptr(zr), ptr(q), ptr(h), ptr(drh), ptr(dq),
                                    ptr(dzr), ptr(dh), stream_of(h)), f"dro_gru_backward_elem({stage})")


@_gru_elem_op.register_fake
def _(stage, dhn, zr, q, h, drh, dq, dzr, dh):
    return None


@torch.library.custom_op("dro::convgru_candidate_backward", mutates_args=("dzr", "dh", "grad_srcs"))
def _gru_cand_bwd_op(srcs: list[Tensor], weight: Tensor, dq: Tensor, zr: Tensor, h: Tensor, dzr: Tensor,
                     dh: Tensor, grad_srcs: list[Tensor], accumulate: list[int]) -> None:
    lib = _lib.load()
    hd, Cin, KH, KW = weight.shape
    B, _, H, W = srcs[0].shape
    tgt = [None] + [g if g.numel() else None for g in grad_srcs[1:]]
    ws, nws = _workspace(B, H, W, Cin, hd, KH, KW, dq.device)
    ptrs, ctot, coff = _grad_targets(tgt) if any(t is not None for t in tgt) else (None, None, None)
    acc = (ctypes.c_int * len(srcs))(*accumulate) if ptrs is not None else None
    check(lib.dro_convgru_candidate_backward(_slices(srcs), len(srcs), ptr(weight), B, H, W, hd, KH, KW,
                                             ptr(dq.contiguous()), ptr(zr), ptr(h), ptr(dzr), ptr(dh), ptrs, ctot,
                                             coff, acc, ptr(ws), nws, stream_of(dq)),
          "dro_convgru_candidate_backward")


@_gru_cand_bwd_op.register_fake
def _(srcs, weight, dq, zr, h, dzr, dh, grad_srcs, accumulate):
    return None


@torch.library.custom_op("dro::convgru_gates_backward",
                         mutates_args=("grad_srcs", "prev_dq", "prev_dzr", "prev_dh"))
def _gru_gates_bwd_op(srcs: list[Tensor], weight: Tensor, dzr: Tensor, grad_srcs: list[Tensor],
                      accumulate: list[int], prev_zr: Tensor, prev_q: Tensor, prev_h: Tensor, prev_dq: Tensor,
                      prev_dzr: Tensor, prev_dh: Tensor, prev_dh_accumulate: int) -> None:
    lib = _lib.load()
    C2, Cin, KH, KW = weight.shape
    B, hd, H, W = srcs[0].shape
    for name, t in (("prev_zr", prev_zr), ("prev_q", prev_q), ("prev_h", prev_h), ("prev_dq", prev_dq),
                    ("prev_dzr", prev_dzr), ("prev_dh", prev_dh)):
        if not t.is_contiguous():
            raise RuntimeError(f"convgru_gates_backward: {name} must be contiguous")
    tgt = [g if g.numel() else None for g in grad_srcs]
    ws, nws = _workspace(B, H, W, Cin, C2, KH, KW, dzr.device)
    ptrs, ctot, coff = _grad_targets(tgt)
    acc = (ctypes.c_int * len(srcs))(*accumulate)
    check(lib.dro_convgru_gates_backward(_slices(srcs), len(srcs), ptr(weight), B, H, W, hd, KH, KW,
                                         ptr(dzr.contiguous()), ptrs, ctot, coff, acc, ptr(prev_zr), ptr(prev_q),
                                         ptr(prev_h), ptr(prev_dq), ptr(prev_dzr), ptr(prev_dh),
                                         int(prev_dh_accumulate), ptr(ws), nws, stream_of(dzr)),
          "dro_convgru_gates_backward")


@_gru_gates_bwd_op.register_fake
def _(srcs, weight, dzr, grad_srcs, accumulate, prev_zr, prev_q, prev_h, prev_dq, prev_dzr, prev_dh,
      prev_dh_accumulate):
    return None


_GRU_FOLD = os.environ.get("DRO_GRU_FOLD", "1") != "0"
_GRU_CHAIN = _GRU_FOLD and os.environ.get("DRO_GRU_CHAIN", "1") != "0"


class GruChain:
    __slots__ = ("first", "hn_ptr", "direct", "zr", "q", "h", "hsink", "done", "dq", "dzr", "dh", "h_in_sink")
    folded = 0
    stats = {"first": 0, "second": 0, "linked": 0, "bwd_linked": 0}

    def __init__(self):
        self.first = False
        self.done = False
        self.hn_ptr = None


_SEPGRU_CHAIN = []


@torch.library.custom_op("dro::sepconvgru_half", mutates_args=())
def _sepgru_op(h: Tensor, wz: Tensor, bz: Tensor, wr: Tensor, br: Tensor, wq: Tensor, bq: Tensor, xs: list[Tensor],
               wzr: Optional[Tensor], bzr: Optional[Tensor]) -> tuple[Tensor, Tensor, Tensor, Tensor]:
    lib = _lib.load()
    require_device(h, wz, wq, *xs, what="sepconvgru")
    h = h.contiguous()
    B, hd, H, W = h.shape
    KH, KW = wz.shape[2:]
    cin = wz.shape[1]
    if wzr is None:
        wzr = torch.cat([wz, wr], 0).contiguous()
        bzr = torch.cat([bz, br], 0).contiguous()
    st = stream_of(h)
    zr = torch.empty(B, 2 * hd, H, W, device=h.device)
    rh = torch.empty_like(h)
    ws, nws = _workspace(B, H, W, cin, 2 * hd, KH, KW, h.device)
    wq = wq.contiguous()
    zf, zb = _wsplit(wzr)
    qf, qb = _wsplit(wq)
    check(lib.dro_convgru_gates_forward(_slices([h, *xs]), 1 + len(xs), ptr(wzr), ptr(bzr), B, H, W, hd,
                                        KH, KW, ptr(zr), ptr(rh), ptr(zf), ptr(ws), nws, st),
          "dro_convgru_gates_forward")
    q = torch.empty_like(h)
    hn = torch.empty_like(h)
    z_sl = DroSlice(zr.data_ptr(), hd, 2 * hd, 0, 0)
    h_sl = DroSlice(h.data_ptr(), hd, hd, 0, 0)
    wsq, nwsq = _workspace(B, H, W, cin, hd, KH, KW, h.device)
    check(lib.dro_convgru_blend_forward(_slices([rh, *xs]), 1 + len(xs), ptr(wq), ptr(bq),
                                        B, H, W, hd, KH, KW, ctypes.byref(z_sl), ctypes.byref(h_sl),
                                        ptr(q), ptr(hn), hd, 0, ptr(qf), ptr(wsq), nwsq, st),
          "dro_convgru_blend_forward")
    return hn, zr, rh, q


@_sepgru_op.register_fake
def _(h, wz, bz, wr, br, wq, bq, xs, wzr, bzr):
    B, hd, H, W = h.shape
    return h.new_empty(h.shape), h.new_empty((B, 2 * hd, H, W)), h.new_empty(h.shape), h.new_empty(h.shape)


def _sepgru_setup(ctx, inputs, output):
    h, wz, bz, wr, br, wq, bq, xs, wzr_in, bzr_in = inputs
    hn, zr, rh, q = output
    wzr = wzr_in if wzr_in is not None else torch.cat([wz, wr], 0).detach().contiguous()
    ctx.wsplit = (_wsplit_bwd(wzr), _wsplit_bwd(wq.contiguous()))
    hc = h.contiguous()
    ctx.save_for_backward(hc, rh, wzr, wq.contiguous(), zr, q, *xs)
    ctx.mark_non_differentiable(zr, rh, q)
    ctx.set_materialize_grads(False)
    ctx.sinks = [_sink_of(x) if x.requires_grad else None for x in xs]
    ctx.hsink = _sink_of(h) if h.requires_grad else None
    ctx.need = (h.requires_grad, [x.requires_grad for x in xs],
                any(t.requires_grad for t in (wz, bz, wr, br)), any(t.requires_grad for t in (wq, bq)))
    ctx.scope = current_scope()
    ctx.keys = (("zr", wz.data_ptr(), wr.data_ptr()), ("q", wq.data_ptr()))
    ctx.direct = _SEPGRU_DIRECT.pop() if _SEPGRU_DIRECT else None
    chain = _SEPGRU_CHAIN.pop() if _SEPGRU_CHAIN else None
    ctx.chain_first = ctx.chain_prev = None
    if chain is not None and _GRU_CHAIN:
        GruChain.stats["second" if chain.first else "first"] += 1
        if not chain.first:
            chain.first = True
            chain.hn_ptr = hn.data_ptr()
            chain.direct = ctx.direct is not None
            chain.zr, chain.q, chain.h, chain.hsink = zr, q, hc, ctx.hsink
            ctx.chain_first = chain
        elif chain.hn_ptr == h.data_ptr() and chain.direct and ctx.direct is not None and h.requires_grad:
            ctx.chain_prev = chain
            GruChain.stats["linked"] += 1


_SEPGRU_DIRECT = []


def _sepgru_backward(ctx, dhn, _gzr, _grh, _gq):
    h, rh, wzr, wq, zr, q, *xs = ctx.saved_tensors
    B, hd, H, W = h.shape
    need_h, need_x, need_zr_w, need_q_w = ctx.need
    if dhn is None:
        return (None,) * 7 + ([None] * len(xs), None, None)
    dhn = dhn.contiguous()
    first = ctx.chain_first
    if first is not None and first.done:
        dq, dzr, dh, h_in_sink = first.dq, first.dzr, first.dh, first.h_in_sink
        first.dq = first.dzr = first.dh = first.zr = first.q = first.h = first.hsink = None
        first.done = False
    else:
        dq = torch.empty_like(h)
        h_in_sink = ctx.hsink is not None and not ctx.hsink.written
        dh = ctx.hsink.target()[0] if h_in_sink else torch.empty_like(h)
        dzr = torch.empty_like(zr)
        torch.ops.dro.gru_backward_elem(1, dhn, zr, q, h, None, dq, dzr, dh)
    drh = torch.empty_like(h)
    sinks = ctx.sinks
    dxs = [torch.empty(B, x.shape[1], H, W, device=h.device) if need_x[i] and sinks[i] is None
           else None for i, x in enumerate(xs)]
    sk = [sn.target() if sn is not None else (None, 0) for sn in sinks]
    tg = [t if sn is not None else d for (t, _), sn, d in zip(sk, sinks, dxs)]
    qacc0 = [0] + [a for _, a in sk]
    zb, qb = ctx.wsplit
    nones = (None,) * 6
    if ctx.direct is not None:
        (_, _), (gwzr, gbzr), (gwq, gbq) = ctx.direct
        if _GRU_FOLD and qb is None:
            torch.ops.dro.convgru_candidate_backward([rh, *xs], wq, dq, zr, h, dzr, dh,
                                                     [_placeholder(t, h.device) for t in [None, *tg]], qacc0)
        else:
            _conv_bwd([rh, *xs], wq, None, dq, 0, 1.0, [drh, *tg], qacc0, wsplit=qb)
        if not _queue_weight_grad([rh, *xs], wq.shape, 0, 1.0, dq, None, gwq, gbq):
            _conv_bwd([rh, *xs], wq, None, dq, 0, 1.0, [None] * (1 + len(xs)), [0] * (1 + len(xs)), gwq, gbq, 1)
        if not (_GRU_FOLD and qb is None):
            torch.ops.dro.gru_backward_elem(2, None, zr, None, h, drh, None, dzr, dh)
        p = ctx.chain_prev
        if p is not None:
            GruChain.stats["bwd_linked"] += 1
        if p is not None and p.h is None:
            p = None
        if p is not None and zb is None:
            p.dq, p.dzr = torch.empty_like(p.h), torch.empty_like(p.zr)
            if p.hsink is not None:
                p.dh, pacc = p.hsink.target()
                p.h_in_sink = True
            else:
                p.dh, pacc, p.h_in_sink = torch.empty_like(p.h), 0, False
            torch.ops.dro.convgru_gates_backward([h, *xs], wzr, dzr, [dh, *[_placeholder(t, h.device) for t in tg]],
                                                 [1] * (1 + len(xs)), p.zr, p.q, p.h, p.dq, p.dzr, p.dh, pacc)
            p.done = True
            GruChain.folded += 1
        else:
            _conv_bwd([h, *xs], wzr, None, dzr, 0, 1.0, [dh, *tg], [1] * (1 + len(xs)), wsplit=zb)
        if not _queue_weight_grad([h, *xs], wzr.shape, 0, 1.0, dzr, None, gwzr, gbzr):
            _conv_bwd([h, *xs], wzr, None, dzr, 0, 1.0, [None] * (1 + len(xs)), [0] * (1 + len(xs)), gwzr, gbzr, 1)
        return (dh if need_h and not h_in_sink else None, *nones, dxs, None, None)
    gwq, gbq, qacc, qfirst = _grad_buffers(ctx.scope, ctx.keys[1], wq, hd, h.device)
    _conv_bwd([rh, *xs], wq, None, dq, 0, 1.0, [drh, *tg], qacc0, gwq, gbq, qacc, qb)
    torch.ops.dro.gru_backward_elem(2, None, zr, None, h, drh, None, dzr, dh)
    gwzr, gbzr, zacc, zfirst = _grad_buffers(ctx.scope, ctx.keys[0], wzr, 2 * hd, h.device)
    _conv_bwd([h, *xs], wzr, None, dzr, 0, 1.0, [dh, *tg], [1] * (1 + len(xs)), gwzr, gbzr, zacc, zb)
    gz = (gwzr[:hd], gbzr[:hd], gwzr[hd:], gbzr[hd:]) if (zfirst and need_zr_w) else (None,) * 4
    gq = (gwq, gbq) if (qfirst and need_q_w) else (None, None)
    return (dh if need_h and not h_in_sink else None, *gz, *gq, dxs, None, None)


torch.library.register_autograd("dro::sepconvgru_half", _sepgru_backward, setup_context=_sepgru_setup)


def sepconvgru_half(h, convz, convr, convq, xs, chain=None):
    direct = None
    zr = _direct_targets((convz.weight, convr.weight), (convz.bias, convr.bias), mark=False)
    if zr is not None:
        qd = _direct_targets((convq.weight,), (convq.bias,), mark=False)
        if qd is not None:
            direct = ((zr[0], zr[1]), (zr[2], zr[3]), (qd[2], qd[3]))
            _mark_direct([convz.weight, convz.bias, convr.weight, convr.bias, convq.weight, convq.bias])
    scope = current_scope()
    if direct is not None:
        wzr, bzr = direct[0]
    else:
        key = ("zr", convz.weight.data_ptr(), convr.weight.data_ptr())
        ent = scope.cats.get(key) if scope is not None else None
        if ent is None:
            ent = (torch.cat([convz.weight, convr.weight], 0).detach().contiguous(),
                   torch.cat([convz.bias, convr.bias], 0).detach().contiguous())
            if scope is not None:
                scope.cats[key] = ent
        wzr, bzr = ent
    _SEPGRU_DIRECT[:] = [direct] if direct is not None else []
    _SEPGRU_CHAIN[:] = [chain] if chain is not None else []
    try:
        return torch.ops.dro.sepconvgru_half(h, convz.weight, convz.bias, convr.weight, convr.bias, convq.weight,
                                             convq.bias, list(xs), wzr, bzr)[0]
    finally:
        _SEPGRU_DIRECT.clear()
        _SEPGRU_CHAIN.clear()
```

dro-sfm_amd/networks/depth_pose/DepthPoseNet.py:

```python
import contextlib
import os
import logging

import torch
import torch.nn as nn

from ... import hip
from ...hip.timeline import stamp, stamp_grad
from ..optim.extractor import ResNetEncoder
from ..optim.update import (BasicUpdateBlockDepth, BasicUpdateBlockPose, DepthHead, PoseHead,
                            UpMaskNet)


def _null():
    return contextlib.nullcontext()


def parse_version(version):
    assert version and "it" in version, f"bad DepthPoseNet version {version!r}"
    fields = version.split("-")
    total = int(fields[0].split("it")[1])
    seq = next((int(f.split("seq")[1]) for f in fields if "seq" in f), 4)
    return {"outer": total // seq, "seq": seq, "high": "h" in version,
            "out_norm": "out" in version, "inter": "inter" in version}


_SIDE_STREAMS = {}

_CL_REFS = os.environ.get("DRO_CL_REFS", "1") != "0"


_CONCURRENT_BLOCKS = [True]


def set_concurrent_blocks(enabled):
    _CONCURRENT_BLOCKS[0] = bool(enabled)


def _pose_stream(device, name="pose"):
    st = _SIDE_STREAMS.get((device, name))
    if st is None:
        prio = 0
        if os.environ.get("DRO_STREAM_PRIO", "0") == "1":
            lo, hi = torch.cuda.Stream.priority_range()
            prio = hi if name == "pose" else lo
        st = _SIDE_STREAMS[(device, name)] = torch.cuda.Stream(device=device, priority=prio)
    return st


_CNET_DEPTH_STREAM = [os.environ.get("DRO_CNET_DEPTH_STREAM", "pose")]


def set_cnet_depth_stream(mode):
    if mode not in ("pose", "own"):
        raise ValueError(mode)
    _CNET_DEPTH_STREAM[0] = mode


class DepthPoseNet(nn.Module):
    def __init__(self, version=None, min_depth=0.1, max_depth=100, **kwargs):
        super().__init__()
        cfg = parse_version(version)
        self.version = version
        self.min_depth, self.max_depth = min_depth, max_depth
        self.iters, self.seq_len = cfg["outer"], cfg["seq"]
        self.is_high, self.out_normalize, self.inter_sup = cfg["high"], cfg["out_norm"], cfg["inter"]
        logging.info("DepthPoseNet(%s): outer=%d seq=%d inter=%s high=%s out_norm=%s", version,
                     self.iters, self.seq_len, self.inter_sup, self.is_high, self.out_normalize)
        self.foutput_dim, self.feat_ratio = 128, 8
        self.hdim, self.cdim = (128 if self.is_high else 64), 32
        C, r, hd, cd = self.foutput_dim, self.feat_ratio, self.hdim, self.cdim
        self.fnet = ResNetEncoder(out_chs=C, stride=r)
        self.depth_head = DepthHead(input_dim=C, hidden_dim=C, scale=False)
        self.pose_head = PoseHead(input_dim=2 * C, hidden_dim=C)
        self.upmask_net = UpMaskNet(hidden_dim=C, ratio=r)
        self.update_block_depth = BasicUpdateBlockDepth(hidden_dim=hd, cost_dim=C, ratio=r, context_dim=cd)
        self.update_block_pose = BasicUpdateBlockPose(hidden_dim=hd, cost_dim=C, context_dim=cd)
        self.cnet = ResNetEncoder(out_chs=C, stride=r)
        self.cnet_depth = ResNetEncoder(out_chs=hd + cd, stride=r, num_input_images=1)
        self.cnet_pose = ResNetEncoder(out_chs=hd + cd, stride=r, num_input_images=2)
        for name in ("fnet", "cnet", "cnet_depth", "cnet_pose"):
            if hasattr(self, name):
                enc = getattr(self, name)
                object.__setattr__(enc, "_dro_tag", name)
                for mname, m in enc.named_modules():
                    if isinstance(m, nn.BatchNorm2d):
                        object.__setattr__(m, "_dro_tag", f"{name}.{mname}")
        for mname, m in self.named_modules():
            if isinstance(m, nn.Conv2d):
                object.__setattr__(m, "_dro_tag", mname)

    @property
    def depth_mode(self):
        return hip.DEPTH_DISP if self.out_normalize else hip.DEPTH_INV

    def scale_inv_depth(self, disp):
        if not self.out_normalize:
            return disp
        lo, hi = 1.0 / self.max_depth, 1.0 / self.min_depth
        return lo + (hi - lo) * disp

    def upsample_depth(self, depth, mask, ratio=8):
        return hip.convex_upsample(depth, mask, ratio)

    def upsample_scaled(self, depth, mask, ratio=8):
        if not self.out_normalize:
            return hip.convex_upsample(depth, mask, ratio)
        lo, hi = 1.0 / self.max_depth, 1.0 / self.min_depth
        return hip.convex_upsample(depth, mask, ratio, affine=(lo, hi - lo))

    def upsample_many(self, pairs, ratio=8):
        affine = None
        if self.out_normalize:
            lo, hi = 1.0 / self.max_depth, 1.0 / self.min_depth
            affine = (lo, hi - lo)
        disps, masks = zip(*pairs)
        return list(hip.convex_upsample_many(list(disps), list(masks), ratio, affine=affine).unbind(0))

    def _cost(self, fmap1, frefs, disp, poses, K, reduce_mean, tag=None):
        return hip.warp_cost(fmap1, frefs, disp, poses, K, depth_mode=self.depth_mode,
                             min_depth=self.min_depth, max_depth=self.max_depth,
                             scale=1.0 / self.feat_ratio, reduce_mean=reduce_mean, tag=tag)

    def forward(self, target_image, ref_imgs, intrinsics):
        with hip.weight_grad_scope():
            return self._forward(target_image, ref_imgs, intrinsics)

    def _forward(self, target_image, ref_imgs, intrinsics):
        B, N = target_image.shape[0], len(ref_imgs)
        C, hd, cd = self.foutput_dim, self.hdim, self.cdim
        K = intrinsics.float().contiguous()
        stamp("fwd:begin")

        cuda = target_image.is_cuda
        pside = None
        if self.iters > 0 and _CONCURRENT_BLOCKS[0] and cuda:
            pside = _pose_stream(target_image.device)
        d_stream = p_stream = None
        d_event = None
        if self.iters > 0 and cuda:
            if pside is not None:
                p_stream = d_stream = pside
                if _CNET_DEPTH_STREAM[0] == "own":
                    d_stream = _pose_stream(target_image.device, "cnet_depth")
            main = torch.cuda.current_stream(target_image.device)
            for st in {d_stream, p_stream} - {None}:
                st.wait_stream(main)
                for t in [target_image, *ref_imgs]:
                    t.record_stream(st)
        if self.iters > 0:
            with torch.cuda.stream(d_stream) if d_stream is not None else _null():
                ctx_d = stamp_grad(self.cnet_depth(target_image), "bwd:cnet_depth_begin")
                h_d, x_d = torch.split(ctx_d, [hd, cd], 1)
                h_d, x_d = torch.tanh(h_d), torch.relu(x_d)
                hip.ops.record_branch(("relu_seq", "ctx_d"), lambda: (x_d > 0).to(torch.uint8), x_d)
                stamp("fwd:cnet_depth")
                if d_stream is not None:
                    d_event = torch.cuda.Event()
                    d_event.record(d_stream)
            with torch.cuda.stream(p_stream) if p_stream is not None else _null():
                pairs = torch.cat([target_image.unsqueeze(0).expand(N, *target_image.shape),
                                   torch.stack(list(ref_imgs))], 2).flatten(0, 1)
                ctx_p = stamp_grad(self.cnet_pose(pairs), "bwd:cnet_pose_begin")
                h_p, x_p = torch.split(ctx_p, [hd, cd], 1)
                h_p, x_p = torch.tanh(h_p), torch.relu(x_p)
                hip.ops.record_branch(("relu_seq", "ctx_p"), lambda: (x_p > 0).to(torch.uint8), x_p)
                stamp("fwd:cnet_pose")

        fmaps = stamp_grad(self.fnet(torch.cat([target_image] + list(ref_imgs), 0)), "bwd:fnet_begin")
        stamp("fwd:fnet")
        assert target_image.shape[2] // fmaps.shape[2] == self.feat_ratio
        h, w = fmaps.shape[2:]
        fmap1_raw, frefs_raw = torch.split(fmaps, [B, N * B], 0)
        frefs_raw = frefs_raw.view(N, B, C, h, w)
        frefs_cl = hip.ops.channels_last_refs(frefs_raw) if _CL_REFS else frefs_raw
        fmap1, frefs = hip.grad_sink(fmap1_raw), hip.grad_sink(frefs_cl)

        pair = torch.cat([fmap1.unsqueeze(0).expand(N, B, C, h, w), frefs_raw], 2).view(N * B, 2 * C, h, w)
        poses = self.pose_head(pair).view(N, B, 6)

        disp = stamp_grad(self.depth_head(fmap1, act_fn=torch.sigmoid), "bwd:init_depth_head")
        up_pairs = [(disp, self.upmask_net(fmap1))]
        stamp("fwd:init_heads")
        pose_preds = [poses]

        main = torch.cuda.current_stream(target_image.device) if cuda else None
        if d_stream is not None:
            if d_event is not None:
                main.wait_event(d_event)
            else:
                main.wait_stream(d_stream)
            for t in (h_d, x_d):
                t.record_stream(main)
        if p_stream is not None and p_stream is not pside:
            main.wait_stream(p_stream)
            for t in (h_p, x_p):
                t.record_stream(main)

        fmap1_p, frefs_p = fmap1, frefs
        if self.iters > 0:
            x_d = hip.grad_sink(x_d)
            if pside is None:
                x_p = hip.grad_sink(x_p)
            else:
                main = torch.cuda.current_stream(target_image.device)
                pside.wait_stream(main)
                with torch.cuda.stream(pside):
                    x_p = hip.grad_sink(x_p)
                    fmap1_p, frefs_p = hip.grad_sink(fmap1_raw), hip.grad_sink(frefs_cl)
        for it in range(self.iters):
            disp = disp.detach()
            poses = poses.detach()
            frozen_poses, frozen_disp = poses, disp

            def depth_block(h_d):
                depth_cost = lambda d: self._cost(fmap1, frefs, d, frozen_poses, K, True, ("depth", it))
                h_d, masks, disps = self.update_block_depth(h_d, depth_cost, frozen_disp, x_d,
                                                            seq_len=self.seq_len)
                keep = range(self.seq_len) if self.inter_sup else [self.seq_len - 1]
                for k in keep:
                    up_pairs.append((disps[k], masks[k]))
                stamp(f"fwd:depth_iter{it}")
                return stamp_grad(h_d, f"bwd:depth_iter{it}"), disps[-1]

            def pose_block(h_p):
                pose_cost = lambda q: self._cost(fmap1_p, frefs_p, frozen_disp, q.view(N, B, 6), K,
                                                 False, ("pose", it)).view(N * B, C, h, w)
                h_p, seq = self.update_block_pose(h_p, pose_cost, frozen_poses.reshape(N * B, 6), x_p,
                                                  seq_len=self.seq_len)
                seq = seq if self.inter_sup else [seq[-1]]
                stamp(f"fwd:pose_iter{it}")
                return stamp_grad(h_p, f"bwd:pose_iter{it}"), [q.view(N, B, 6) for q in seq]

            if pside is None:
                h_d, disp_last = depth_block(h_d)
                h_p, seq = pose_block(h_p)
            else:
                main = torch.cuda.current_stream(target_image.device)
                pside.wait_stream(main)
                for t in (fmap1_p, frefs_p, frozen_disp, frozen_poses, h_p, x_p, K):
                    t.record_stream(pside)
                with torch.cuda.stream(pside):
                    h_p, seq = pose_block(h_p)
                h_d, disp_last = depth_block(h_d)
                main.wait_stream(pside)
                for t in (h_p, *seq):
                    t.record_stream(main)
            pose_preds.extend(seq)
            disp, poses = disp_last, seq[-1]

        if not self.training:
            return self.upsample_scaled(*up_pairs[-1], self.feat_ratio), pose_preds[-1].permute(1, 0, 2)
        if cuda:
            inv_preds = self.upsample_many(up_pairs, self.feat_ratio)
            stamp("fwd:upsample")
        else:
            inv_preds = [self.upsample_scaled(d, m, self.feat_ratio) for d, m in up_pairs]
        return inv_preds, torch.stack(pose_preds, 2).permute(1, 0, 2, 3)
```

dro-sfm_amd/networks/optim/update.py:

```python
import torch
import torch.nn as nn
import torch.nn.functional as F

from ... import hip
from ...hip import conv as hip_conv

_BACKEND = "hip"
_ACT_FN = {None: lambda x: x, "relu": F.relu, "sigmoid": torch.sigmoid, "tanh": torch.tanh}


def set_conv_backend(name):
    global _BACKEND
    if name not in ("hip", "miopen"):
        raise ValueError(name)
    _BACKEND = name


def conv_backend():
    return _BACKEND


def declare(module, table):
    for name, (cin, cout, k, pad) in table.items():
        setattr(module, name, nn.Conv2d(cin, cout, k, padding=pad))


def _as_list(x):
    return list(x) if isinstance(x, (list, tuple)) else [x]


def conv(srcs, weight, bias, act=None, alpha=1.0):
    srcs = _as_list(srcs)
    if _BACKEND == "hip":
        return hip.conv2d(srcs, weight, bias, act=act, alpha=alpha)
    kh, kw = weight.shape[2:]
    x = srcs[0] if len(srcs) == 1 else torch.cat(srcs, 1)
    y = _ACT_FN[act](F.conv2d(x, weight, bias, padding=(kh // 2, kw // 2)))
    return y * alpha if alpha != 1.0 else y


def conv_cat(x, convs, act=None):
    if _BACKEND == "hip":
        y = hip.conv2d(_as_list(x), None, None, act=act,
                       parts=(tuple(c.weight for c in convs), tuple(c.bias for c in convs)))
    else:
        y = conv(x, torch.cat([c.weight for c in convs], 0), torch.cat([c.bias for c in convs], 0), act)
    return torch.split(y, [c.out_channels for c in convs], 1)


relu_rec = hip.ops.record_relu


def fused_groups(*convs):
    return [[c.weight for c in convs], [c.bias for c in convs]]


def mask_seq(hidden_dim, ratio):
    return nn.Sequential(nn.Conv2d(hidden_dim, 2 * hidden_dim, 3, padding=1), nn.ReLU(inplace=True),
                         nn.Conv2d(2 * hidden_dim, 9 * ratio * ratio, 1, padding=0))


class DepthHead(nn.Module):

    def __init__(self, input_dim=256, hidden_dim=128, scale=False):
        super().__init__()
        self.scale = scale
        declare(self, {"conv1": (input_dim, hidden_dim, 3, 1), "conv2": (hidden_dim, 1, 3, 1)})

    def forward(self, x_d, act_fn=torch.tanh):
        act = {torch.tanh: "tanh", torch.sigmoid: "sigmoid"}.get(act_fn)
        y = conv(relu_rec(conv(x_d, self.conv1.weight, self.conv1.bias, "relu"), self.conv1),
                 self.conv2.weight, self.conv2.bias, act)
        return y if act is not None else act_fn(y)


class PoseHead(nn.Module):

    def __init__(self, input_dim=256, hidden_dim=128):
        super().__init__()
        declare(self, {"conv1_pose": (input_dim, hidden_dim, 3, 1),
                       "conv2_pose": (hidden_dim, 6, 3, 1)})
        self.register_buffer("_scale", torch.tensor([[1.0, 1.0, 1.0, 0.01, 0.01, 0.01]]),
                             persistent=False)

    def forward(self, x_p, pose=None):
        y = conv(relu_rec(conv(x_p, self.conv1_pose.weight, self.conv1_pose.bias, "relu"), self.conv1_pose),
                 self.conv2_pose.weight, self.conv2_pose.bias)
        return hip.pose_mean(y, 0.01, pose)


class SepConvGRU(nn.Module):

    def __init__(self, hidden_dim=128, input_dim=192 + 128):
        super().__init__()
        cin = hidden_dim + input_dim
        self.hidden_dim = hidden_dim
        for axis, k, pad in (("1", (1, 5), (0, 2)), ("2", (5, 1), (2, 0))):
            declare(self, {g + axis: (cin, hidden_dim, k, pad) for g in ("convz", "convr", "convq")})

    def _gate(self, h, xs, axis, chain=None):
        cz, cr, cq = (getattr(self, g + axis) for g in ("convz", "convr", "convq"))
        if _BACKEND == "hip":
            return hip.sepconvgru_half(h, cz, cr, cq, xs, chain=chain)
        z, r = conv_cat([h, *xs], (cz, cr), "sigmoid")
        q = conv([r * h, *xs], cq.weight, cq.bias, "tanh")
        return (1 - z) * h + z * q

    def dro_param_groups(self):
        return fused_groups(self.convz1, self.convr1) + fused_groups(self.convz2, self.convr2)

    def forward(self, h, x):
        xs = _as_list(x)
        chain = hip_conv.GruChain() if _BACKEND == "hip" else None
        return self._gate(self._gate(h, xs, "1", chain), xs, "2", chain)


class _Projection(nn.Module):

    def __init__(self, tag, state_ch, cost_dim, hidden_dim, out_chs):
        super().__init__()
        self.out_chs, self._tag = out_chs, tag
        declare(self, {"convc1": (cost_dim, hidden_dim, 1, 0),
                       "convc2": (hidden_dim, hidden_dim, 3, 1),
                       f"conv{tag}1": (state_ch, hidden_dim, 7, 3),
                       f"conv{tag}2": (hidden_dim, 64, 3, 1),
                       f"conv{tag}": (64 + hidden_dim, out_chs - state_ch, 3, 1)})

    def sources(self, state_map, cost):
        t = self._tag
        c1, c2 = self.convc1, self.convc2
        s1, s2, f = (getattr(self, f"conv{t}{i}") for i in ("1", "2", ""))
        cor = relu_rec(conv(relu_rec(conv(cost, c1.weight, c1.bias, "relu"), c1), c2.weight, c2.bias, "relu"), c2)
        sfm = relu_rec(conv(relu_rec(conv(state_map, s1.weight, s1.bias, "relu"), s1), s2.weight, s2.bias, "relu"),
                       s2)
        return [hip.grad_sink(relu_rec(conv([cor, sfm], f.weight, f.bias, "relu"), f)), state_map]


class ProjectionInputDepth(_Projection):
    def __init__(self, cost_dim, hidden_dim, out_chs):
        super().__init__("d", 1, cost_dim, hidden_dim, out_chs)

    def forward(self, depth, cost):
        return torch.cat(self.sources(depth, cost), 1)


class ProjectionInputPose(_Projection):
    def __init__(self, cost_dim, hidden_dim, out_chs):
        super().__init__("p", 6, cost_dim, hidden_dim, out_chs)

    def pose_map(self, pose, cost):
        bs, _, h, w = cost.shape
        return pose.reshape(bs, 6, 1, 1).expand(bs, 6, h, w)

    def sources(self, pose, cost):
        return super().sources(hip.grad_sink(self.pose_map(pose, cost)), cost)

    def forward(self, pose, cost):
        return torch.cat(self.sources(pose, cost), 1)


class UpMaskNet(nn.Module):

    def __init__(self, hidden_dim=128, ratio=8):
        super().__init__()
        self.mask = mask_seq(hidden_dim, ratio)

    def forward(self, feat):
        m0, m2 = self.mask[0], self.mask[2]
        return conv(relu_rec(conv(feat, m0.weight, m0.bias, "relu"), m0), m2.weight, m2.bias, None, 0.25)


class BasicUpdateBlockDepth(nn.Module):

    def __init__(self, hidden_dim=128, cost_dim=256, ratio=8, context_dim=64):
        super().__init__()
        self.encoder = ProjectionInputDepth(cost_dim=cost_dim, hidden_dim=hidden_dim, out_chs=hidden_dim)
        self.depth_gru = SepConvGRU(hidden_dim=hidden_dim, input_dim=hidden_dim + context_dim)
        self.depth_head = DepthHead(hidden_dim, hidden_dim=hidden_dim, scale=False)
        self.mask = mask_seq(hidden_dim, ratio)

    def dro_param_groups(self):
        return fused_groups(self.depth_head.conv1, self.mask[0])

    def heads(self, net):
        a, b = conv_cat(net, (self.depth_head.conv1, self.mask[0]), "relu")
        a, b = relu_rec(a, self.depth_head.conv1), relu_rec(b, self.mask[0])
        c2, m2 = self.depth_head.conv2, self.mask[2]
        return conv(a, c2.weight, c2.bias, "tanh"), conv(b, m2.weight, m2.bias, None, 0.25)

    def forward(self, net, cost_func, inv_depth, context, seq_len=4, scale_func=None):
        scale_func = scale_func or (lambda x: (x, None))
        invs, masks = [], []
        for _ in range(seq_len):
            inv_depth = hip.grad_sink(inv_depth)
            feat = self.encoder.sources(inv_depth, cost_func(scale_func(inv_depth)[0]))
            net = hip.grad_sink(self.depth_gru(net, [context, *feat]))
            delta, mask = self.heads(net)
            inv_depth = inv_depth + delta
            invs.append(inv_depth)
            masks.append(mask)
        return net, masks, invs


class BasicUpdateBlockPose(nn.Module):

    def __init__(self, hidden_dim=128, cost_dim=256, context_dim=64):
        super().__init__()
        self.encoder = ProjectionInputPose(cost_dim=cost_dim, hidden_dim=hidden_dim, out_chs=hidden_dim)
        self.pose_gru = SepConvGRU(hidden_dim=hidden_dim, input_dim=hidden_dim + context_dim)
        self.pose_head = PoseHead(hidden_dim, hidden_dim=hidden_dim)

    def forward(self, net, cost_func, pose, inp, seq_len=4):
        seq = []
        for _ in range(seq_len):
            net = hip.grad_sink(self.pose_gru(net, [inp, *self.encoder.sources(pose, cost_func(pose))]))
            pose = self.pose_head(net, pose)
            seq.append(pose)
        return net, seq
```

include/dro_amd.h:

```cpp
#ifndef DRO_AMD_H
#define DRO_AMD_H

#include <stddef.h>

#ifdef __cplusplus
extern "C" {
#endif

#define DRO_POSE_EULER 0
#define DRO_POSE_MATRIX 1

#define DRO_DEPTH_METRIC 0
#define DRO_DEPTH_INV 1
#define DRO_DEPTH_DISP 2

#define DRO_OK 0
#define DRO_E_NULL (-1)
#define DRO_E_SHAPE (-2)
#define DRO_E_MODE (-3)

const char* dro_last_error(void);
int dro_abi_version(void);

int dro_timestamp(unsigned long long* buf, int slot, void* stream);
// ... 37 lines not shown

size_t dro_photometric_clip_offset(int B, int N, int n, int H, int W, int which);

int dro_photometric_forward(const float* image, const float* context, const float* inv_depths,
                            const float* K, const float* ref_K, const float* pose, int pose_mode,
                            int B, int N, int n, int H, int W,
                            float ssim_w, float C1, float C2, float smooth_w,
                            int automask, int reduce_min, float clip_loss,
                            float* out, void* workspace, void* stream);

int dro_photometric_backward(const float* image, const float* context, const float* inv_depths,
                             const float* K, const float* ref_K, const float* pose, int pose_mode,
                             int B, int N, int n, int H, int W,
                             float ssim_w, float C1, float C2, float smooth_w,
                             int automask, int reduce_min, float clip_loss,
                             const float* grad_out, float* grad_inv_depths, float* grad_pose,
                             void* workspace, int* cells, signed char* l1_signs, void* stream);

size_t dro_supervised_workspace_bytes(int B, int N, int n, int H, int W);

int dro_supervised_forward(const float* gt_inv, const float* inv_depths, const float* K,
                           const float* ref_K, const float* gt_pose, const float* pose,
                           int pose_mode, int B, int N, int n, int H, int W,
                           float min_depth, float max_depth, float* out,
                           void* workspace, void* stream);

int dro_supervised_backward(const float* gt_inv, const float* inv_depths, const float* K,
                            const float* ref_K, const float* gt_pose, const float* pose,
                            int pose_mode, int B, int N, int n, int H, int W,
                            float min_depth, float max_depth, const float* grad_out,
                            float* grad_inv_depths, float* grad_pose, void* workspace,
                            void* stream);

int dro_convex_upsample_forward(const float* inv, const float* mask, int B, int h, int w,
                                int ratio, float add, float mul, float* out, void* stream);
int dro_convex_upsample_backward(const float* inv, const float* mask, const float* grad_out,
                                 int B, int h, int w, int ratio, float mul,
                                 float* grad_inv, float* grad_mask, void* stream);
int dro_convex_upsample_many_forward(const float* const* inv, const float* const* mask, int n, int B,
                                     int h, int w, int ratio, float add, float mul, float* out,
                                     void* stream);
size_t dro_convex_upsample_many_workspace_bytes(int n, int B, int h, int w);
int dro_convex_upsample_many_backward(const float* const* inv, const float* const* mask,
                                      const float* grad_out, int n, int B, int h, int w, int ratio,
                                      float mul, float* const* grad_inv, float* const* grad_mask,
                                      void* workspace, size_t workspace_bytes, void* stream);

int dro_bilinear_upsample2x_forward(const float* x, long long planes, int h, int w,
                                    float* out, void* stream);
int dro_bilinear_upsample2x_backward(const float* grad_out, long long planes, int h, int w,
                                     float* grad_x, void* stream);

int dro_maxpool3x3s2_forward(const float* x, long long planes, int H, int W, float* y,
                             unsigned char* argmax, void* stream);
int dro_maxpool3x3s2_backward(const float* grad_y, const unsigned char* argmax,
                              long long planes, int H, int W, float* grad_x, void* stream);

int dro_depth_metrics_blocks(int H, int W);
size_t dro_depth_metrics_workspace_bytes(int B);
int dro_depth_metrics_prepare(const float* gt, const float* pred, int B, int H, int W, int h, int w,
                              float min_depth, float max_depth, int crop_y1, int crop_y2,
                              int crop_x1, int crop_x2, float* pred_up, float* ratio,
                              int* block_counts, void* stream);
size_t dro_depth_metrics_median_workspace_bytes(int B);
int dro_depth_metrics_median(const float* ratio, const int* block_counts, int B, int H, int W,
                             float* scale, void* workspace, void* stream);
int dro_depth_metrics_reduce(const float* gt, const float* pred_up, const float* scale, int B, int H,
                             int W, float min_depth, float max_depth, int crop_y1, int crop_y2,
                             int crop_x1, int crop_x2, float* metrics, void* workspace, void* stream);

int dro_depth_metrics_demon_prepare(const float* gt, const float* pred, const float* gt_pose,
                                    long long pose_stride, int B, int H, int W, int h, int w,
                                    float min_depth, float max_depth, float* pred_up, float* ratio,
                                    int* block_counts, void* stream);
int dro_depth_metrics_demon_reduce(const float* gt, const float* pred_up, const float* scale,
                                   const float* gt_pose, long long pose_stride, int B, int H, int W,
                                   float min_depth, float max_depth, float* metrics, void* workspace,
                                   void* stream);

int dro_post_process_inv_depth(const float* inv, const float* inv_flipped, int B, int H, int W,
                               int method, float* inv_pp, float* depth, float* depth_pp, void* stream);

int dro_resize_rgb8_to_tensor(const unsigned char* src, int N, int H0, int W0, int H, int W,
                              const int* xbounds, const int* xcoef, int KX, const int* ybounds,
                              const int* ycoef, int KY, unsigned char* tmp, float* dst, void* stream);

int dro_resize_rgb8(const unsigned char* src, int N, int H0, int W0, int H, int W,
                    const int* xbounds, const int* xcoef, int KX, const int* ybounds,
                    const int* ycoef, int KY, unsigned char* tmp, unsigned char* dst, void* stream);
int dro_rgb8_to_tensor(const unsigned char* src, int N, int H, int W, float* dst, void* stream);

size_t dro_png_filtered_bytes(int H, int W, int bpp);
int dro_png_decode(const unsigned char* zdata, const long long* zoff, int N, int H, int W, int kind,
                   unsigned char* filtered, void* out, int* status, void* stream);
int dro_color_jitter_rgb8(unsigned char* frames, int N, int H, int W, const int* params,
                          unsigned long long* workspace, void* stream);

size_t dro_batchnorm_workspace_bytes(int N, int C, int HW);
int dro_batchnorm_relu_forward(const float* x, const float* gamma, const float* beta,
                               const float* skip, int relu, int N, int C, int HW, float eps,
                               float momentum, float* running_mean, float* running_var,
                               long long* num_batches_tracked, float* y, float* save_mean,
                               float* save_invstd, void* workspace, size_t workspace_bytes,
                               void* stream);
int dro_batchnorm_relu_backward(const float* grad_out, const float* x, const float* y,
                                const float* gamma, const float* save_mean,
                                const float* save_invstd, int relu, int N, int C, int HW,
                                float* grad_x, float* grad_gamma, float* grad_beta,
                                float* grad_skip, void* workspace, size_t workspace_bytes,
                                void* stream);

typedef struct dro_slice {
  const float* data;
  int channels;
  int total_channels;
  int channel_offset;
  int broadcast;
} dro_slice;

#define DRO_ACT_NONE 0
#define DRO_ACT_RELU 1
#define DRO_ACT_SIGMOID 2
#define DRO_ACT_TANH 3

size_t dro_weight_split_bytes(int Cout, int Cin, int KH, int KW, int transposed);
int dro_weight_split(const float* weight, int Cout, int Cin, int KH, int KW, void* fwd, void* bwd,
                     void* stream);

size_t dro_conv2d_workspace_bytes(int B, int H, int W, int Cin, int Cout, int KH, int KW);

int dro_conv2d_plan(int rows, int kch, int KH, int KW, int B, int H, int W, long long* info);

int dro_debug_conv_stamps(void* buffer);

int dro_conv_log(int enable);
long long dro_conv_log_read(char* buf, long long cap);

int dro_conv2d_forward(const dro_slice* srcs, int nsrc, const float* weight, const float* bias,
                       int B, int H, int W, int Cout, int KH, int KW, int act, float alpha,
                       float* out, int out_ctot, int out_coff, const void* wsplit,
                       void* workspace, size_t workspace_bytes, void* stream);

int dro_convgru_gates_forward(const dro_slice* srcs, int nsrc, const float* weight,
                              const float* bias, int B, int H, int W, int hd, int KH, int KW,
                              float* zr, float* rh, const void* wsplit, void* workspace,
                              size_t workspace_bytes, void* stream);

int dro_convgru_blend_forward(const dro_slice* srcs, int nsrc, const float* weight,
                              const float* bias, int B, int H, int W, int Cout, int KH, int KW,
                              const dro_slice* z, const dro_slice* h, float* q_out, float* out,
                              int out_ctot, int out_coff, const void* wsplit, void* workspace,
                              size_t workspace_bytes, void* stream);

int dro_conv2d_backward(const dro_slice* srcs, int nsrc, const float* weight, int B, int H, int W,
                        int Cout, int KH, int KW, int act, float alpha, const dro_slice* y,
                        const float* dout, float* const* grad_srcs, const int* grad_ctot,
                        const int* grad_coff, const int* grad_accumulate, float* grad_weight,
                        float* grad_bias, int grad_weight_accumulate, const void* wsplit,
                        void* workspace, size_t workspace_bytes, void* stream);

size_t dro_conv2d_strided_workspace_bytes(int B, int Hi, int Wi, int Cin, int Cout, int KH, int KW,
                                          int stride, int pad);
int dro_conv2d_strided_forward(const float* x, const float* weight, const float* bias, int B, int Hi,
                               int Wi, int Cin, int Cout, int KH, int KW, int stride, int pad, int act,
                               float* out, void* workspace, size_t workspace_bytes, void* stream);
int dro_conv2d_strided_backward(const float* x, const float* weight, const float* dout, int B, int Hi,
                                int Wi, int Cin, int Cout, int KH, int KW, int stride, int pad,
                                float* grad_x, int grad_x_accumulate, float* grad_weight,
                                float* grad_bias, int grad_weight_accumulate, void* workspace,
                                size_t workspace_bytes, void* stream);

int dro_pose_mean_forward(const float* y, const float* pose, float* out, int B, int C, int HW,
                          float rot_scale, void* stream);
int dro_pose_mean_backward(const float* gout, float* gy, int B, int C, int HW, float rot_scale,
                           void* stream);

typedef struct dro_wgrad_use {
  const dro_slice* srcs;
  const float* dout;
  const float* y;
} dro_wgrad_use;

size_t dro_conv2d_weight_grad_multi_workspace_bytes(int nuse, int B, int H, int W, int Cin, int Cout,
                                                    int KH, int KW);

int dro_conv2d_weight_grad_multi(const dro_wgrad_use* uses, int nuse, int nsrc, int B, int H, int W,
                                 int Cout, int KH, int KW, int act, float alpha, float* grad_weight,
                                 float* grad_bias, int accumulate, void* workspace,
                                 size_t workspace_bytes, void* stream);

typedef struct dro_wgrad_member {
  const dro_wgrad_use* uses;
  int nuse;
  int nsrc;
  int B, H, W, Cout;
  float alpha;
  float* grad_weight;
  float* grad_bias;
  int accumulate;
} dro_wgrad_member;

int dro_conv2d_weight_grad_group_capacity(int* max_members, int* max_uses);

size_t dro_conv2d_weight_grad_group_workspace_bytes(const dro_wgrad_member* members, int nmember,
                                                    int KH, int KW);

int dro_conv2d_weight_grad_group(const dro_wgrad_member* members, int nmember, int KH, int KW,
                                 int act, void* workspace, size_t workspace_bytes, void* stream);

int dro_gru_backward_elem(int stage, int B, int hd, int H, int W, const float* dhn,
                          const float* zr, const float* q, const float* h, const float* drh,
                          float* dq, float* dzr, float* dh, void* stream);

int dro_convgru_candidate_backward(const dro_slice* srcs, int nsrc, const float* weight, int B, int H, int W,
                                   int hd, int KH, int KW, const float* dq, const float* zr, const float* h,
                                   float* dzr, float* dh, float* const* grad_srcs, const int* grad_ctot,
                                   const int* grad_coff, const int* grad_accumulate, void* workspace,
                                   size_t workspace_bytes, void* stream);

int dro_convgru_gates_backward(const dro_slice* srcs, int nsrc, const float* weight, int B, int H, int W,
                               int hd, int KH, int KW, const float* dzr_in, float* const* grad_srcs,
                               const int* grad_ctot, const int* grad_coff, const int* grad_accumulate,
                               const float* prev_zr, const float* prev_q, const float* prev_h, float* prev_dq,
                               float* prev_dzr, float* prev_dh, int prev_dh_accumulate, void* workspace,
                               size_t workspace_bytes, void* stream);

typedef struct dro_bn_params {
  const float* gamma;
  const float* beta;
  float* running_mean;
  float* running_var;
  long long* num_batches_tracked;
  float eps, momentum;
  float* save_mean;
  float* save_invstd;
} dro_bn_params;

typedef struct dro_bn_grad_params {
  const float* y;
  const float* z;
  const float* gamma;
  const float* save_mean;
  const float* save_invstd;
  float* grad_gamma;
  float* grad_beta;
} dro_bn_grad_params;

size_t dro_bn_state_bytes(int B, int H, int W, int C);

int dro_bn_apply(const float* x, const float* skip, int relu, int B, int C, int H, int W, const void* state,
                 float* y, void* stream);

int dro_bn_backward_apply(const float* g, const float* z, int B, int C, int H, int W, const void* state,
                          float* dz, void* stream);

int dro_conv2d_bn_forward(const float* x, int B, int H, int W, int Cin, const float* weight, int Cout,
                          const void* in_state, const float* in_skip, float* in_y,
                          const dro_bn_params* bn, void* out_state, float* out, void* workspace,
                          size_t workspace_bytes, void* stream);

int dro_conv2d_bn_backward_data(const float* weight, int B, int H, int W, int Cin, int Cout, const float* dout,
                                const void* gin_state, const float* gin_z, float* gin_dz,
                                const dro_bn_grad_params* src_bn, void* src_state, float* grad_x,
                                int grad_x_accumulate, void* workspace, size_t workspace_bytes, void* stream);

int dro_adam_step(float* param, const float* grad, float* exp_avg, float* exp_avg_sq, long long n,
                  const float* step, const float* hyper, void* stream);

#ifdef __cplusplus
}
#endif
#endif
```

Measured before the change: 141.8 images/s.

## Precompute loop-invariant context projection for ConvGRU gates and skip its channels per iteration

The context features fed to every SepConvGRU step do not change across iterations, so their contribution to the z/r/q convolutions is computed once per forward by a new context-projection kernel. The per-step gate and blend kernels then skip that channel range (a 'hole' in the K loop) and seed accumulators, or the split-K reduction, with the precomputed partial sums. This removes repeated GEMM work over the context channels in each of the seq_len x iters GRU calls. In exchange it adds extra buffers, stream-lifetime bookkeeping, and constraints on chunk alignment; the backward path still has to supply gradients for the context input.

```diff
diff --git a/dro-sfm_amd/csrc/conv.hip b/dro-sfm_amd/csrc/conv.hip
--- a/dro-sfm_amd/csrc/conv.hip
+++ b/dro-sfm_amd/csrc/conv.hip
@@ -355,7 +355,10 @@
   const int ty0 = tyi * TH, tx0 = (trem - tyi * a.tiles_x) * TW;
   const size_t HW = (size_t)H * W;
   const unsigned HWu = (unsigned)HW;
-  const int nck = (kch + CK - 1) / CK;
+  constexpr bool HOLE = MODE == 0 && XF == 0 && EPI <= 2;
+  const int hole_beg = HOLE ? a.hole_beg : 0, hole_len = HOLE ? a.hole_len : 0;
+  const int nck = HOLE && a.hole_nck ? a.hole_nck : (kch + CK - 1) / CK;
+  auto phys = [&](int l) { return HOLE ? l + (l >= hole_beg ? hole_len : 0) : l; };
   const int cbeg = blockIdx.y * a.chunks_per_split;
   const int cend = min(nck, cbeg + a.chunks_per_split);
 
@@ -427,7 +430,7 @@
   };
   constexpr int NVM = WPER4 + XPER * NJ;
   auto prep = [&](Stage& st, int chunk, Rows& r) {
-    const int c0 = chunk * CK;
+    const int c0 = phys(chunk) * CK;
     r.gbase = MODE == 0 ? (unsigned)row0 * CinT + (unsigned)c0 * T : (unsigned)c0 * CinT + (unsigned)row0 * T;
     unsigned cm = 0;
 #pragma unroll
@@ -536,7 +539,6 @@
   f32x16 acc;
 #pragma unroll
   for (int r = 0; r < 16; ++r) acc[r] = 0.f;
-
   const int nit = (cend - cbeg + KS - 1) / KS;
   auto chunk_of = [&](int it) { return cbeg + it * KS + grp; };
   unsigned long long* const stp = a.stamps ? a.stamps + (size_t)blockIdx.x * 16 : nullptr;
@@ -582,6 +584,20 @@
   if (chunk_of(0) < cend) {
     load(sa, chunk_of(0));
     store(sa, 0);
+  }
+  constexpr bool PRE_ACC = HOLE && (EPI == 1 || EPI == 2) && KS == 4;
+  constexpr bool PRE_RED = HOLE && (EPI == 1 || EPI == 2) && KS < 4;
+  if constexpr (PRE_ACC) {
+    if (a.pre && grp == 0 && wk == 0 && blockIdx.y == 0) {
+      const int oy = ty0 + qy, ox = tx0 + qx;
+      const bool pok = oy < H && ox < W;
+      const float* pp = a.pre + (size_t)b * rows * HW + (pok ? (size_t)oy * W + ox : 0);
+#pragma unroll
+      for (int r = 0; r < 16; ++r) {
+        const int row = row0 + wr * 32 + (r & 3) + 8 * (r >> 2) + 4 * hi;
+        if (pok && row < rows) acc[r] = pp[(size_t)row * HW];
+      }
+    }
   }
   stamp(12);
   if (PF == 2 && chunk_of(1) < cend) load(sb, chunk_of(1));
@@ -697,7 +713,15 @@
   }
   for (int e = threadIdx.x; e < BM * 64; e += 256 * KS) {
     const int rl = e >> 6, pl = e & 63;
+    const int row = row0 + rl;
+    const int py = pl / TW, px = pl - py * TW;
+    const int oy = ty0 + py, ox = tx0 + px;
+    if (row >= rows || oy >= H || ox >= W) continue;
+    const size_t epix = (size_t)oy * W + ox;
     float v = 0.f;
+    if constexpr (PRE_RED) {
+      if (a.pre && blockIdx.y == 0) v = a.pre[((size_t)b * rows + row) * HW + epix];
+    }
 #pragma unroll
     for (int g = 0; g < KS; ++g) {
       if (WM == 1)
@@ -705,11 +729,6 @@
       else
         v += smem_all[((size_t)g * BM + rl) * 64 + pl];
     }
-    const int row = row0 + rl;
-    const int py = pl / TW, px = pl - py * TW;
-    const int oy = ty0 + py, ox = tx0 + px;
-    if (row >= rows || oy >= H || ox >= W) continue;
-    const size_t epix = (size_t)oy * W + ox;
     if (a.part)
       a.part[(size_t)blockIdx.y * rows * P + (size_t)row * P + (size_t)b * HW + epix] = v;
     else
@@ -2360,8 +2379,12 @@
 
 unsigned long long* g_conv_stamps = nullptr;
 
+struct ChanHole {
+  int c0, cn, only;
+};
+
 template <int MODE, int ACT, int EPI, int XF = 0>
-int launch_igemm(IgArgs& a, long long P, char* ws, hipStream_t s) {
+int launch_igemm(IgArgs& a, long long P, char* ws, hipStream_t s, const ChanHole* hole = nullptr) {
   IgPlan pl = a.flat_only ? plan_igemm_flat(a.rows, a.kch, a.g.KH, a.g.KW, a.g.B, a.g.H, a.g.W)
                           : plan_igemm(a.rows, a.kch, a.g.KH, a.g.KW, a.g.B, a.g.H, a.g.W);
   constexpr bool BNF = EPI >= 5 || XF != 0;
@@ -2382,6 +2405,29 @@
     a.dbg = e ? atoi(e) : 0;
   }
   a.K = a.kch * a.g.KH * a.g.KW;
+  a.hole_beg = a.hole_len = a.hole_nck = 0;
+  int kch_run = a.kch;
+  if (hole) {
+    bool ok = MODE == 0 && XF == 0 && EPI <= 2 && pl.halo && !a.flat_only && !a.wsplit && hole->c0 >= 0 &&
+              hole->cn >= 1 && hole->c0 + hole->cn <= a.kch && hole->c0 % pl.CK == 0 && hole->cn % pl.CK == 0;
+    if constexpr (MODE == 0 && EPI <= 2) ok = ok && !thin_ok<MODE, EPI>(a);
+    const int nfull = ok ? (a.kch + pl.CK - 1) / pl.CK : 0, nhole = ok ? hole->cn / pl.CK : 0;
+    if (!ok || (!hole->only && nhole >= nfull)) {
+      set_error("conv2d: the channel hole must be whole chunks of an f32 halo-kernel launch "
+                "(offset and length multiples of 16 channels for 1x5 / 5x1)");
+      return DRO_E_MODE;
+    }
+    a.hole_beg = hole->only ? 0 : hole->c0 / pl.CK;
+    a.hole_len = hole->only ? hole->c0 / pl.CK : nhole;
+    a.hole_nck = hole->only ? nhole : nfull - nhole;
+    kch_run = hole->only ? hole->cn : a.kch - hole->cn;
+    while (pl.kin > 1 && pl.kin > a.hole_nck) pl.kin >>= 1;
+    int ks = pl.ksplit;
+    if (ks > a.hole_nck / pl.kin) ks = a.hole_nck / pl.kin;
+    if (ks < 1) ks = 1;
+    pl.chunks_per_split = (a.hole_nck + ks - 1) / ks;
+    pl.ksplit = (a.hole_nck + pl.chunks_per_split - 1) / pl.chunks_per_split;
+  }
   static const bool thin_off = getenv("DRO_CONV_NO_THIN") != nullptr;
   if (!BNF && !a.flat_only && !thin_off && thin_ok<MODE, EPI>(a)) {
     a.part = reinterpret_cast<float*>(ws);
@@ -2394,7 +2440,7 @@
   a.chunks_per_split = pl.chunks_per_split;
   a.part = pl.ksplit > 1 ? reinterpret_cast<float*>(ws) : nullptr;
   const dim3 grid(pl.row_tiles * pl.ptiles, pl.ksplit);
-  const double flops = 2.0 * a.rows * a.kch * a.g.KH * a.g.KW * (double)P;
+  const double flops = 2.0 * a.rows * kch_run * a.g.KH * a.g.KW * (double)P;
   if (pl.halo)
     conv_logf(flops, "dconv_kernel<%d, %d, %d, %d, %d, %d, %d>", pl.bm, a.g.KH, a.g.KW, MODE, ACT, EPI, pl.kin);
   else
@@ -2852,11 +2898,13 @@
   return launch_igemm<1, 0, 0, 0>(a, P, ws, s);
 }
 
-extern "C" int dro_convgru_gates_forward(const dro_slice* srcs, int nsrc, const float* weight,
-                                         const float* bias, int B, int H, int W, int hd, int KH, int KW,
-                                         float* zr, float* rh, const void* wsplit, void* workspace,
-                                         size_t workspace_bytes, void* stream) {
+static int convgru_gates_forward_impl(const dro_slice* srcs, int nsrc, const float* weight,
+                                      const float* bias, int B, int H, int W, int hd, int KH, int KW,
+                                      float* zr, float* rh, const void* wsplit, void* workspace,
+                                      size_t workspace_bytes, void* stream, const float* pre,
+                                      const ChanHole* hole) {
   IgArgs a = {};
+  a.pre = pre;
   a.wsplit = static_cast<const char*>(wsplit);
   int st = conv_setup_geom(a, srcs, nsrc, B, H, W, 2 * hd, KH, KW);
   if (st) return st;
@@ -2882,15 +2930,40 @@
   a.hd = hd;
   a.rows = 2 * hd;
   a.kch = a.g.Cin;
-  return launch_igemm<0, 2, 2>(a, (long long)B * H * W, static_cast<char*>(workspace), (hipStream_t)stream);
-}
-
-extern "C" int dro_convgru_blend_forward(const dro_slice* srcs, int nsrc, const float* weight,
-                                         const float* bias, int B, int H, int W, int Cout, int KH, int KW,
-                                         const dro_slice* z, const dro_slice* h, float* q_out, float* out,
-                                         int out_ctot, int out_coff, const void* wsplit, void* workspace,
+  return launch_igemm<0, 2, 2>(a, (long long)B * H * W, static_cast<char*>(workspace), (hipStream_t)stream,
+                               hole);
+}
+
+extern "C" int dro_convgru_gates_forward(const dro_slice* srcs, int nsrc, const float* weight,
+                                         const float* bias, int B, int H, int W, int hd, int KH, int KW,
+                                         float* zr, float* rh, const void* wsplit, void* workspace,
                                          size_t workspace_bytes, void* stream) {
+  return convgru_gates_forward_impl(srcs, nsrc, weight, bias, B, H, W, hd, KH, KW, zr, rh, wsplit, workspace,
+                                    workspace_bytes, stream, nullptr, nullptr);
+}
+
+extern "C" int dro_convgru_gates_forward_ctx(const dro_slice* srcs, int nsrc, const float* weight,
+                                             const float* bias, int B, int H, int W, int hd, int KH, int KW,
+                                             float* zr, float* rh, const float* pre, int hole_c0,
+                                             int hole_cn, void* workspace, size_t workspace_bytes,
+                                             void* stream) {
+  if (!srcs || !weight || !zr || !rh || !pre) {
+    set_error("convgru_gates_forward_ctx: NULL srcs/weight/zr/rh/pre");
+    return DRO_E_NULL;
+  }
+  const ChanHole hole = {hole_c0, hole_cn, 0};
+  return convgru_gates_forward_impl(srcs, nsrc, weight, bias, B, H, W, hd, KH, KW, zr, rh, nullptr, workspace,
+                                    workspace_bytes, stream, pre, &hole);
+}
+
+static int convgru_blend_forward_impl(const dro_slice* srcs, int nsrc, const float* weight,
+                                      const float* bias, int B, int H, int W, int Cout, int KH, int KW,
+                                      const dro_slice* z, const dro_slice* h, float* q_out, float* out,
+                                      int out_ctot, int out_coff, const void* wsplit, void* workspace,
+                                      size_t workspace_bytes, void* stream, const float* pre,
+                                      const ChanHole* hole) {
   IgArgs a = {};
+  a.pre = pre;
   a.wsplit = static_cast<const char*>(wsplit);
   int st = conv_setup_geom(a, srcs, nsrc, B, H, W, Cout, KH, KW);
   if (st) return st;
@@ -2913,7 +2986,69 @@
   a.rows = Cout;
   a.kch = a.g.Cin;
   return launch_igemm<0, 3, 1>(a, (long long)B * H * W, static_cast<char*>(workspace),
-                               (hipStream_t)stream);
+                               (hipStream_t)stream, hole);
+}
+
+extern "C" int dro_convgru_blend_forward(const dro_slice* srcs, int nsrc, const float* weight,
+                                         const float* bias, int B, int H, int W, int Cout, int KH, int KW,
+                                         const dro_slice* z, const dro_slice* h, float* q_out, float* out,
+                                         int out_ctot, int out_coff, const void* wsplit, void* workspace,
+                                         size_t workspace_bytes, void* stream) {
+  return convgru_blend_forward_impl(srcs, nsrc, weight, bias, B, H, W, Cout, KH, KW, z, h, q_out, out, out_ctot,
+                                    out_coff, wsplit, workspace, workspace_bytes, stream, nullptr, nullptr);
+}
+
+extern "C" int dro_convgru_blend_forward_ctx(const dro_slice* srcs, int nsrc, const float* weight,
+                                             const float* bias, int B, int H, int W, int Cout, int KH, int KW,
+                                             const dro_slice* z, const dro_slice* h, float* q_out, float* out,
+                                             int out_ctot, int out_coff, const float* pre, int hole_c0,
+                                             int hole_cn, void* workspace, size_t workspace_bytes,
+                                             void* stream) {
+  if (!srcs || !weight || !z || !h || !z->data || !h->data || !q_out || !out || !pre) {
+    set_error("convgru_blend_forward_ctx: NULL srcs/weight/z/h/q/out/pre");
+    return DRO_E_NULL;
+  }
+  const ChanHole hole = {hole_c0, hole_cn, 0};
+  return convgru_blend_forward_impl(srcs, nsrc, weight, bias, B, H, W, Cout, KH, KW, z, h, q_out, out, out_ctot,
+                                    out_coff, nullptr, workspace, workspace_bytes, stream, pre, &hole);
+}
+
+extern "C" int dro_convgru_context_proj_forward(const dro_slice* ctx, const float* weight, int B, int H, int W,
+                                                int Cout, int Cin, int c_off, int KH, int KW, float* out,
+                                                void* workspace, size_t workspace_bytes, void* stream) {
+  if (!ctx || !ctx->data || !weight || !out) {
+    set_error("convgru_context_proj_forward: NULL ctx/weight/out");
+    return DRO_E_NULL;
+  }
+  IgArgs a = {};
+  int st = conv_setup_geom(a, ctx, 1, B, H, W, Cout, KH, KW);
+  if (st) return st;
+  const int cn = ctx->channels;
+  if (c_off < 0 || Cin < 1 || c_off + cn > Cin || Cin >= 4096 || (long long)Cin * KH * KW >= 65535 ||
+      too_big(B, Cin > Cout ? Cin : Cout, (long long)H * W)) {
+    set_error("convgru_context_proj_forward: the context channels do not fit the weight's Cin");
+    return DRO_E_SHAPE;
+  }
+  if ((st = check_ws(workspace, workspace_bytes, fwd_workspace(B, H, W, Cin, Cout, KH, KW),
+                     "convgru_context_proj_forward")))
+    return st;
+  a.g.Cin = Cin;
+  a.cindiv = make_fdiv(Cin);
+  a.src[1] = a.src[0];
+  a.cbase[0] = 0;
+  a.cbase[1] = c_off;
+  a.cbase[2] = a.cbase[3] = c_off + cn;
+  a.weight = weight;
+  a.bias = nullptr;
+  a.alpha = 1.f;
+  a.out = out;
+  a.out_ctot = Cout;
+  a.out_coff = 0;
+  a.rows = Cout;
+  a.kch = Cin;
+  const ChanHole hole = {c_off, cn, 1};
+  return launch_igemm<0, 0, 0>(a, (long long)B * H * W, static_cast<char*>(workspace), (hipStream_t)stream,
+                               &hole);
 }
 
 struct GruFold {
diff --git a/dro-sfm_amd/csrc/conv_common.hpp b/dro-sfm_amd/csrc/conv_common.hpp
--- a/dro-sfm_amd/csrc/conv_common.hpp
+++ b/dro-sfm_amd/csrc/conv_common.hpp
@@ -121,6 +121,8 @@
   unsigned long long* stamps;
   int dbg;
   BnFuse bn;
+  const float* pre;
+  int hole_beg, hole_len, hole_nck;
 };
 
 #ifndef DRO_CONV_ABLATE
diff --git a/dro-sfm_amd/hip/_lib.py b/dro-sfm_amd/hip/_lib.py
--- a/dro-sfm_amd/hip/_lib.py
+++ b/dro-sfm_amd/hip/_lib.py
@@ -88,6 +88,9 @@
     _sig(lib.dro_conv2d_forward, P, I, P, P, I, I, I, I, I, I, I, F, P, I, I, P, P, Z, S)
     _sig(lib.dro_convgru_gates_forward, P, I, P, P, I, I, I, I, I, I, P, P, P, P, Z, S)
     _sig(lib.dro_convgru_blend_forward, P, I, P, P, I, I, I, I, I, I, P, P, P, P, I, I, P, P, Z, S)
+    _sig(lib.dro_convgru_context_proj_forward, P, P, I, I, I, I, I, I, I, I, P, P, Z, S)
+    _sig(lib.dro_convgru_gates_forward_ctx, P, I, P, P, I, I, I, I, I, I, P, P, P, I, I, P, Z, S)
+    _sig(lib.dro_convgru_blend_forward_ctx, P, I, P, P, I, I, I, I, I, I, P, P, P, P, I, I, P, I, I, P, Z, S)
     _sig(lib.dro_conv2d_backward, P, I, P, I, I, I, I, I, I, I, F, P, P, P, P, P, P, P, P, I, P, P, Z, S)
     _sig(lib.dro_conv2d_weight_grad_multi_workspace_bytes, I, I, I, I, I, I, I, I, restype=Z)
     _sig(lib.dro_conv2d_weight_grad_multi, P, I, I, I, I, I, I, I, I, I, F, P, P, I, P, Z, S)
@@ -130,6 +133,7 @@
     "dro_weight_split_bytes", "dro_weight_split",
     "dro_conv2d_workspace_bytes", "dro_conv2d_plan", "dro_debug_conv_stamps", "dro_conv_log", "dro_conv_log_read", "dro_conv2d_forward", "dro_convgru_gates_forward",
     "dro_convgru_blend_forward", "dro_conv2d_backward",
+    "dro_convgru_context_proj_forward", "dro_convgru_gates_forward_ctx", "dro_convgru_blend_forward_ctx",
     "dro_conv2d_weight_grad_multi_workspace_bytes", "dro_conv2d_weight_grad_multi",
     "dro_conv2d_weight_grad_group_capacity", "dro_conv2d_weight_grad_group_workspace_bytes",
     "dro_conv2d_weight_grad_group",
diff --git a/dro-sfm_amd/hip/conv.py b/dro-sfm_amd/hip/conv.py
--- a/dro-sfm_amd/hip/conv.py
+++ b/dro-sfm_amd/hip/conv.py
@@ -710,6 +710,10 @@
 @torch.library.custom_op("dro::sepconvgru_half", mutates_args=())
 def _sepgru_op(h: Tensor, wz: Tensor, bz: Tensor, wr: Tensor, br: Tensor, wq: Tensor, bq: Tensor, xs: list[Tensor],
                wzr: Optional[Tensor], bzr: Optional[Tensor]) -> tuple[Tensor, Tensor, Tensor, Tensor]:
+    return _sepgru_run(h, wz, bz, wr, br, wq, bq, xs, wzr, bzr)
+
+
+def _sepgru_run(h, wz, bz, wr, br, wq, bq, xs, wzr, bzr, pzr=None, pq=None, ctx_index=0):
     lib = _lib.load()
     require_device(h, wz, wq, *xs, what="sepconvgru")
     h = h.contiguous()
@@ -724,16 +728,27 @@
     rh = torch.empty_like(h)
     ws, nws = _workspace(B, H, W, cin, 2 * hd, KH, KW, h.device)
     wq = wq.contiguous()
+    q = torch.empty_like(h)
+    hn = torch.empty_like(h)
+    z_sl = DroSlice(zr.data_ptr(), hd, 2 * hd, 0, 0)
+    h_sl = DroSlice(h.data_ptr(), hd, hd, 0, 0)
+    wsq, nwsq = _workspace(B, H, W, cin, hd, KH, KW, h.device)
+    if pzr is not None:
+        c0 = hd + sum(x.shape[1] for x in xs[:ctx_index])
+        cn = xs[ctx_index].shape[1]
+        check(lib.dro_convgru_gates_forward_ctx(_slices([h, *xs]), 1 + len(xs), ptr(wzr), ptr(bzr), B, H, W, hd,
+                                                KH, KW, ptr(zr), ptr(rh), ptr(pzr), c0, cn, ptr(ws), nws, st),
+              "dro_convgru_gates_forward_ctx")
+        check(lib.dro_convgru_blend_forward_ctx(_slices([rh, *xs]), 1 + len(xs), ptr(wq), ptr(bq),
+                                                B, H, W, hd, KH, KW, ctypes.byref(z_sl), ctypes.byref(h_sl),
+                                                ptr(q), ptr(hn), hd, 0, ptr(pq), c0, cn, ptr(wsq), nwsq, st),
+              "dro_convgru_blend_forward_ctx")
+        return hn, zr, rh, q
     zf, zb = _wsplit(wzr)
     qf, qb = _wsplit(wq)
     check(lib.dro_convgru_gates_forward(_slices([h, *xs]), 1 + len(xs), ptr(wzr), ptr(bzr), B, H, W, hd,
                                         KH, KW, ptr(zr), ptr(rh), ptr(zf), ptr(ws), nws, st),
           "dro_convgru_gates_forward")
-    q = torch.empty_like(h)
-    hn = torch.empty_like(h)
-    z_sl = DroSlice(zr.data_ptr(), hd, 2 * hd, 0, 0)
-    h_sl = DroSlice(h.data_ptr(), hd, hd, 0, 0)
-    wsq, nwsq = _workspace(B, H, W, cin, hd, KH, KW, h.device)
     check(lib.dro_convgru_blend_forward(_slices([rh, *xs]), 1 + len(xs), ptr(wq), ptr(bq),
                                         B, H, W, hd, KH, KW, ctypes.byref(z_sl), ctypes.byref(h_sl),
                                         ptr(q), ptr(hn), hd, 0, ptr(qf), ptr(wsq), nwsq, st),
@@ -748,7 +763,8 @@
 
 
 def _sepgru_setup(ctx, inputs, output):
-    h, wz, bz, wr, br, wq, bq, xs, wzr_in, bzr_in = inputs
+    h, wz, bz, wr, br, wq, bq, xs, wzr_in, bzr_in = inputs[:10]
+    ctx.nextra = len(inputs) - 10
     hn, zr, rh, q = output
     wzr = wzr_in if wzr_in is not None else torch.cat([wz, wr], 0).detach().contiguous()
     ctx.wsplit = (_wsplit_bwd(wzr), _wsplit_bwd(wq.contiguous()))
@@ -786,7 +802,7 @@
     B, hd, H, W = h.shape
     need_h, need_x, need_zr_w, need_q_w = ctx.need
     if dhn is None:
-        return (None,) * 7 + ([None] * len(xs), None, None)
+        return (None,) * 7 + ([None] * len(xs), None, None) + (None,) * ctx.nextra
     dhn = dhn.contiguous()
     first = ctx.chain_first
     if first is not None and first.done:
@@ -839,7 +855,7 @@
             _conv_bwd([h, *xs], wzr, None, dzr, 0, 1.0, [dh, *tg], [1] * (1 + len(xs)), wsplit=zb)
         if not _queue_weight_grad([h, *xs], wzr.shape, 0, 1.0, dzr, None, gwzr, gbzr):
             _conv_bwd([h, *xs], wzr, None, dzr, 0, 1.0, [None] * (1 + len(xs)), [0] * (1 + len(xs)), gwzr, gbzr, 1)
-        return (dh if need_h and not h_in_sink else None, *nones, dxs, None, None)
+        return (dh if need_h and not h_in_sink else None, *nones, dxs, None, None) + (None,) * ctx.nextra
     gwq, gbq, qacc, qfirst = _grad_buffers(ctx.scope, ctx.keys[1], wq, hd, h.device)
     _conv_bwd([rh, *xs], wq, None, dq, 0, 1.0, [drh, *tg], qacc0, gwq, gbq, qacc, qb)
     torch.ops.dro.gru_backward_elem(2, None, zr, None, h, drh, None, dzr, dh)
@@ -847,13 +863,98 @@
     _conv_bwd([h, *xs], wzr, None, dzr, 0, 1.0, [dh, *tg], [1] * (1 + len(xs)), gwzr, gbzr, zacc, zb)
     gz = (gwzr[:hd], gbzr[:hd], gwzr[hd:], gbzr[hd:]) if (zfirst and need_zr_w) else (None,) * 4
     gq = (gwq, gbq) if (qfirst and need_q_w) else (None, None)
-    return (dh if need_h and not h_in_sink else None, *gz, *gq, dxs, None, None)
+    return (dh if need_h and not h_in_sink else None, *gz, *gq, dxs, None, None) + (None,) * ctx.nextra
 
 
 torch.library.register_autograd("dro::sepconvgru_half", _sepgru_backward, setup_context=_sepgru_setup)
 
 
-def sepconvgru_half(h, convz, convr, convq, xs, chain=None):
+_CTX_HOIST = os.environ.get("DRO_GRU_CTX_HOIST", "1") != "0"
+_CTX_ALIGN = 16
+CTX_HOIST_CALLS = [0]
+
+
+@torch.library.custom_op("dro::gru_context_proj", mutates_args=())
+def _gru_ctx_proj_op(context: Tensor, wzr: Tensor, wq: Tensor, c_off: int) -> tuple[Tensor, Tensor]:
+    lib = _lib.load()
+    require_device(context, wzr, wq, what="gru_context_proj")
+    B, C, H, W = context.shape
+    outs = []
+    for w in (wzr, wq):
+        Cout, Cin, KH, KW = w.shape
+        out = torch.empty(B, Cout, H, W, device=context.device, dtype=torch.float32)
+        ws, nws = _workspace(B, H, W, Cin, Cout, KH, KW, out.device)
+        sl = _slice(context)
+        check(lib.dro_convgru_context_proj_forward(ctypes.byref(sl), ptr(w), B, H, W, Cout, Cin, c_off, KH, KW,
+                                                   ptr(out), ptr(ws), nws, stream_of(out)),
+              "dro_convgru_context_proj_forward")
+        outs.append(out)
+    return outs[0], outs[1]
+
+
+@_gru_ctx_proj_op.register_fake
+def _(context, wzr, wq, c_off):
+    B, _, H, W = context.shape
+    return context.new_empty((B, wzr.shape[0], H, W)), context.new_empty((B, wq.shape[0], H, W))
+
+
+@torch.library.custom_op("dro::sepconvgru_half_ctx", mutates_args=())
+def _sepgru_ctx_op(h: Tensor, wz: Tensor, bz: Tensor, wr: Tensor, br: Tensor, wq: Tensor, bq: Tensor,
+                   xs: list[Tensor], wzr: Optional[Tensor], bzr: Optional[Tensor], pzr: Tensor, pq: Tensor,
+                   ctx_index: int) -> tuple[Tensor, Tensor, Tensor, Tensor]:
+    return _sepgru_run(h, wz, bz, wr, br, wq, bq, xs, wzr, bzr, pzr, pq, ctx_index)
+
+
+@_sepgru_ctx_op.register_fake
+def _(h, wz, bz, wr, br, wq, bq, xs, wzr, bzr, pzr, pq, ctx_index):
+    B, hd, H, W = h.shape
+    return h.new_empty(h.shape), h.new_empty((B, 2 * hd, H, W)), h.new_empty(h.shape), h.new_empty(h.shape)
+
+
+torch.library.register_autograd("dro::sepconvgru_half_ctx", _sepgru_backward, setup_context=_sepgru_setup)
+
+
+class GruCtxProj:
+    __slots__ = ("context", "halves")
+
+    def __init__(self, context):
+        self.context = context
+        self.halves = {}
+
+
+def _fused_zr(convz, convr, direct):
+    if direct is not None:
+        return direct[0]
+    scope = current_scope()
+    key = ("zr", convz.weight.data_ptr(), convr.weight.data_ptr())
+    ent = scope.cats.get(key) if scope is not None else None
+    if ent is None:
+        ent = (torch.cat([convz.weight, convr.weight], 0).detach().contiguous(),
+               torch.cat([convz.bias, convr.bias], 0).detach().contiguous())
+        if scope is not None:
+            scope.cats[key] = ent
+    return ent
+
+
+def gru_context_proj(context, halves, hidden_dim):
+    cd = context.shape[1]
+    if (not _CTX_HOIST or _XCONV[0] or not context.is_cuda or hidden_dim % _CTX_ALIGN or cd % _CTX_ALIGN
+            or context.stride()[2:] == (0, 0)):
+        return None
+    proj = GruCtxProj(context)
+    with torch.no_grad():
+        for convz, convr, convq in halves:
+            if tuple(convz.weight.shape[2:]) not in ((1, 5), (5, 1)) or convz.weight.shape[1] <= hidden_dim + cd:
+                return None
+            zr = _direct_targets((convz.weight, convr.weight), (convz.bias, convr.bias), mark=False, in_setup=True)
+            qd = _direct_targets((convq.weight,), (convq.bias,), mark=False, in_setup=True) if zr is not None else None
+            wzr = _fused_zr(convz, convr, ((zr[0], zr[1]),) if qd is not None else None)[0]
+            proj.halves[id(convz)] = torch.ops.dro.gru_context_proj(context.detach(), wzr,
+                                                                    convq.weight.detach().contiguous(), hidden_dim)
+    return proj
+
+
+def sepconvgru_half(h, convz, convr, convq, xs, chain=None, ctx_proj=None):
     direct = None
     zr = _direct_targets((convz.weight, convr.weight), (convz.bias, convr.bias), mark=False)
     if zr is not None:
@@ -861,21 +962,20 @@
         if qd is not None:
             direct = ((zr[0], zr[1]), (zr[2], zr[3]), (qd[2], qd[3]))
             _mark_direct([convz.weight, convz.bias, convr.weight, convr.bias, convq.weight, convq.bias])
-    scope = current_scope()
-    if direct is not None:
-        wzr, bzr = direct[0]
-    else:
-        key = ("zr", convz.weight.data_ptr(), convr.weight.data_ptr())
-        ent = scope.cats.get(key) if scope is not None else None
-        if ent is None:
-            ent = (torch.cat([convz.weight, convr.weight], 0).detach().contiguous(),
-                   torch.cat([convz.bias, convr.bias], 0).detach().contiguous())
-            if scope is not None:
-                scope.cats[key] = ent
-        wzr, bzr = ent
+    wzr, bzr = _fused_zr(convz, convr, direct)
+    pre = None
+    if ctx_proj is not None and not _XCONV[0] and h.shape[1] == convq.weight.shape[0]:
+        x0 = xs[0]
+        if x0.data_ptr() == ctx_proj.context.data_ptr() and x0.shape == ctx_proj.context.shape:
+            pre = ctx_proj.halves.get(id(convz))
     _SEPGRU_DIRECT[:] = [direct] if direct is not None else []
     _SEPGRU_CHAIN[:] = [chain] if chain is not None else []
     try:
+        if pre is not None:
+            CTX_HOIST_CALLS[0] += 1
+            return torch.ops.dro.sepconvgru_half_ctx(h, convz.weight, convz.bias, convr.weight, convr.bias,
+                                                     convq.weight, convq.bias, list(xs), wzr, bzr, pre[0], pre[1],
+                                                     0)[0]
         return torch.ops.dro.sepconvgru_half(h, convz.weight, convz.bias, convr.weight, convr.bias, convq.weight,
                                              convq.bias, list(xs), wzr, bzr)[0]
     finally:
diff --git a/dro-sfm_amd/networks/depth_pose/DepthPoseNet.py b/dro-sfm_amd/networks/depth_pose/DepthPoseNet.py
--- a/dro-sfm_amd/networks/depth_pose/DepthPoseNet.py
+++ b/dro-sfm_amd/networks/depth_pose/DepthPoseNet.py
@@ -35,6 +35,10 @@
 
 def set_concurrent_blocks(enabled):
     _CONCURRENT_BLOCKS[0] = bool(enabled)
+
+
+def _proj_tensors(proj):
+    return [t for pair in proj.halves.values() for t in pair] if proj is not None else []
 
 
 def _pose_stream(device, name="pose"):
@@ -138,6 +142,7 @@
             pside = _pose_stream(target_image.device)
         d_stream = p_stream = None
         d_event = None
+        proj_d = proj_p = None
         if self.iters > 0 and cuda:
             if pside is not None:
                 p_stream = d_stream = pside
@@ -154,6 +159,7 @@
                 h_d, x_d = torch.split(ctx_d, [hd, cd], 1)
                 h_d, x_d = torch.tanh(h_d), torch.relu(x_d)
                 hip.ops.record_branch(("relu_seq", "ctx_d"), lambda: (x_d > 0).to(torch.uint8), x_d)
+                proj_d = self.update_block_depth.depth_gru.context_proj(x_d)
                 stamp("fwd:cnet_depth")
                 if d_stream is not None:
                     d_event = torch.cuda.Event()
@@ -165,6 +171,7 @@
                 h_p, x_p = torch.split(ctx_p, [hd, cd], 1)
                 h_p, x_p = torch.tanh(h_p), torch.relu(x_p)
                 hip.ops.record_branch(("relu_seq", "ctx_p"), lambda: (x_p > 0).to(torch.uint8), x_p)
+                proj_p = self.update_block_pose.pose_gru.context_proj(x_p)
                 stamp("fwd:cnet_pose")
 
         fmaps = stamp_grad(self.fnet(torch.cat([target_image] + list(ref_imgs), 0)), "bwd:fnet_begin")
@@ -190,11 +197,11 @@
                 main.wait_event(d_event)
             else:
                 main.wait_stream(d_stream)
-            for t in (h_d, x_d):
+            for t in (h_d, x_d, *_proj_tensors(proj_d)):
                 t.record_stream(main)
         if p_stream is not None and p_stream is not pside:
             main.wait_stream(p_stream)
-            for t in (h_p, x_p):
+            for t in (h_p, x_p, *_proj_tensors(proj_p)):
                 t.record_stream(main)
 
         fmap1_p, frefs_p = fmap1, frefs
@@ -216,7 +223,7 @@
             def depth_block(h_d):
                 depth_cost = lambda d: self._cost(fmap1, frefs, d, frozen_poses, K, True, ("depth", it))
                 h_d, masks, disps = self.update_block_depth(h_d, depth_cost, frozen_disp, x_d,
-                                                            seq_len=self.seq_len)
+                                                            seq_len=self.seq_len, ctx_proj=proj_d)
                 keep = range(self.seq_len) if self.inter_sup else [self.seq_len - 1]
                 for k in keep:
                     up_pairs.append((disps[k], masks[k]))
@@ -227,7 +234,7 @@
                 pose_cost = lambda q: self._cost(fmap1_p, frefs_p, frozen_disp, q.view(N, B, 6), K,
                                                  False, ("pose", it)).view(N * B, C, h, w)
                 h_p, seq = self.update_block_pose(h_p, pose_cost, frozen_poses.reshape(N * B, 6), x_p,
-                                                  seq_len=self.seq_len)
+                                                  seq_len=self.seq_len, ctx_proj=proj_p)
                 seq = seq if self.inter_sup else [seq[-1]]
                 stamp(f"fwd:pose_iter{it}")
                 return stamp_grad(h_p, f"bwd:pose_iter{it}"), [q.view(N, B, 6) for q in seq]
diff --git a/dro-sfm_amd/networks/optim/update.py b/dro-sfm_amd/networks/optim/update.py
--- a/dro-sfm_amd/networks/optim/update.py
+++ b/dro-sfm_amd/networks/optim/update.py
@@ -98,10 +98,10 @@
         for axis, k, pad in (("1", (1, 5), (0, 2)), ("2", (5, 1), (2, 0))):
             declare(self, {g + axis: (cin, hidden_dim, k, pad) for g in ("convz", "convr", "convq")})
 
-    def _gate(self, h, xs, axis, chain=None):
+    def _gate(self, h, xs, axis, chain=None, ctx_proj=None):
         cz, cr, cq = (getattr(self, g + axis) for g in ("convz", "convr", "convq"))
         if _BACKEND == "hip":
-            return hip.sepconvgru_half(h, cz, cr, cq, xs, chain=chain)
+            return hip.sepconvgru_half(h, cz, cr, cq, xs, chain=chain, ctx_proj=ctx_proj)
         z, r = conv_cat([h, *xs], (cz, cr), "sigmoid")
         q = conv([r * h, *xs], cq.weight, cq.bias, "tanh")
         return (1 - z) * h + z * q
@@ -109,10 +109,16 @@
     def dro_param_groups(self):
         return fused_groups(self.convz1, self.convr1) + fused_groups(self.convz2, self.convr2)
 
-    def forward(self, h, x):
+    def context_proj(self, context):
+        if _BACKEND != "hip":
+            return None
+        halves = [tuple(getattr(self, g + axis) for g in ("convz", "convr", "convq")) for axis in ("1", "2")]
+        return hip_conv.gru_context_proj(context, halves, self.hidden_dim)
+
+    def forward(self, h, x, ctx_proj=None):
         xs = _as_list(x)
         chain = hip_conv.GruChain() if _BACKEND == "hip" else None
-        return self._gate(self._gate(h, xs, "1", chain), xs, "2", chain)
+        return self._gate(self._gate(h, xs, "1", chain, ctx_proj), xs, "2", chain, ctx_proj)
 
 
 class _Projection(nn.Module):
@@ -188,13 +194,13 @@
         c2, m2 = self.depth_head.conv2, self.mask[2]
         return conv(a, c2.weight, c2.bias, "tanh"), conv(b, m2.weight, m2.bias, None, 0.25)
 
-    def forward(self, net, cost_func, inv_depth, context, seq_len=4, scale_func=None):
+    def forward(self, net, cost_func, inv_depth, context, seq_len=4, scale_func=None, ctx_proj=None):
         scale_func = scale_func or (lambda x: (x, None))
         invs, masks = [], []
         for _ in range(seq_len):
             inv_depth = hip.grad_sink(inv_depth)
             feat = self.encoder.sources(inv_depth, cost_func(scale_func(inv_depth)[0]))
-            net = hip.grad_sink(self.depth_gru(net, [context, *feat]))
+            net = hip.grad_sink(self.depth_gru(net, [context, *feat], ctx_proj))
             delta, mask = self.heads(net)
             inv_depth = inv_depth + delta
             invs.append(inv_depth)
@@ -210,10 +216,10 @@
         self.pose_gru = SepConvGRU(hidden_dim=hidden_dim, input_dim=hidden_dim + context_dim)
         self.pose_head = PoseHead(hidden_dim, hidden_dim=hidden_dim)
 
-    def forward(self, net, cost_func, pose, inp, seq_len=4):
+    def forward(self, net, cost_func, pose, inp, seq_len=4, ctx_proj=None):
         seq = []
         for _ in range(seq_len):
-            net = hip.grad_sink(self.pose_gru(net, [inp, *self.encoder.sources(pose, cost_func(pose))]))
+            net = hip.grad_sink(self.pose_gru(net, [inp, *self.encoder.sources(pose, cost_func(pose))], ctx_proj))
             pose = self.pose_head(net, pose)
             seq.append(pose)
         return net, seq
diff --git a/include/dro_amd.h b/include/dro_amd.h
--- a/include/dro_amd.h
+++ b/include/dro_amd.h
@@ -213,6 +213,19 @@
                               int out_ctot, int out_coff, const void* wsplit, void* workspace,
                               size_t workspace_bytes, void* stream);
 
+int dro_convgru_context_proj_forward(const dro_slice* ctx, const float* weight, int B, int H, int W,
+                                     int Cout, int Cin, int c_off, int KH, int KW, float* out,
+                                     void* workspace, size_t workspace_bytes, void* stream);
+int dro_convgru_gates_forward_ctx(const dro_slice* srcs, int nsrc, const float* weight,
+                                  const float* bias, int B, int H, int W, int hd, int KH, int KW,
+                                  float* zr, float* rh, const float* pre, int hole_c0, int hole_cn,
+                                  void* workspace, size_t workspace_bytes, void* stream);
+int dro_convgru_blend_forward_ctx(const dro_slice* srcs, int nsrc, const float* weight,
+                                  const float* bias, int B, int H, int W, int Cout, int KH, int KW,
+                                  const dro_slice* z, const dro_slice* h, float* q_out, float* out,
+                                  int out_ctot, int out_coff, const float* pre, int hole_c0,
+                                  int hole_cn, void* workspace, size_t workspace_bytes, void* stream);
+
 int dro_conv2d_backward(const dro_slice* srcs, int nsrc, const float* weight, int B, int H, int W,
                         int Cout, int KH, int KW, int act, float alpha, const dro_slice* y,
                         const float* dout, float* const* grad_srcs, const int* grad_ctot,
```

Measured after the change: 142.0 images/s, median of 5. About the same (+0.1%).
